# pitlover/Monocular-Depth-Estimation

Hardware: AMD Instinct MI355X
Metric: images/sec (train step) NYU 640x480 bs=8/GPU (higher is better)
Workload: dtype fp32; 1 GPU; NewCRFs Swin-L (large07) train step, NYU 480x640; model=NewCRFs-L07, global_batch=8, per_gpu_batch=8, num_accum=1, parallelism=dp1, reference_config=json/nyu/newcrfs/newcrfs_github_eval.json, matmul_precision=fp32, hipgraph=False

## Files before the change

### include/mdemi.h

```cpp
#ifndef MDEMI_H
#define MDEMI_H

#include <stddef.h>
#include <stdint.h>

#ifdef __cplusplus
extern "C" {
#endif

#define MDEMI_OK 0
#define MDEMI_EINVAL (-1)
#define MDEMI_ELAUNCH (-2)
#define MDEMI_EUNSUP (-3)
#define MDEMI_EWORKSPACE (-4)

const char* mdemi_last_error(void);
int mdemi_version(void);


#define MDEMI_L_KCONTIG 0
#define MDEMI_L_MNCONTIG 1
#define MDEMI_L_CONV 2
#define MDEMI_OP_NONE 0
#define MDEMI_OP_GELU 1
#define MDEMI_BIAS_NONE 0
#define MDEMI_BIAS_COL 1
#define MDEMI_BIAS_ROW 2
#define MDEMI_ACT_NONE 0
#define MDEMI_ACT_GELU 1
#define MDEMI_ACT_RELU 2
#define MDEMI_ACT_LEAKY 3
#define MDEMI_ACT_GELU_GRAD 4
#define MDEMI_ACT_SIGMOID 5
#define MDEMI_ACT_SILU 6
#define MDEMI_ACT_RELU_GRAD 7
#define MDEMI_ACT_SILU_GRAD 8
#define MDEMI_PAD_ZERO 0
#define MDEMI_PAD_REPLICATE 1

typedef struct mdemi_conv_geom {
  int32_t n, h, w, c;
  int32_t oh, ow;
  int32_t kh, kw, stride, pad;
  int32_t pad_mode;
  int32_t _reserved;
} mdemi_conv_geom;

typedef struct mdemi_gemm_desc {
  int32_t M, N, K, batch;
  const float* A; int64_t lda; int64_t a_bstride; int32_t a_layout; int32_t a_op;
  const float* B; int64_t ldb; int64_t b_bstride; int32_t b_layout; int32_t b_op;
  float* C; int64_t ldc; int64_t c_bstride;
  float alpha, beta;
  const float* bias; int32_t bias_mode; int32_t act;
  const float* aux; int64_t ldaux; int64_t aux_bstride;
  const float* residual; int64_t ldres; int64_t res_bstride;
  int32_t split_k; int32_t _pad0;
  void* workspace; int64_t workspace_bytes;
  mdemi_conv_geom conv;
  float* preact; int64_t ldpre; int64_t pre_bstride;
  float* rowsum_a;
  int32_t batch_inner; int32_t _pad1;
  int64_t a_bstride_inner, b_bstride_inner, c_bstride_inner;
  const float* row_scale; int64_t row_scale_group;
  const float* m_live; int64_t m_live_group;
  const float* k_live; int64_t k_live_group;
} mdemi_gemm_desc;

size_t mdemi_gemm_workspace_size(const mdemi_gemm_desc* d);
int mdemi_gemm_f32(const mdemi_gemm_desc* d, void* stream);
int mdemi_gemm_f32_pair(const mdemi_gemm_desc* d0, const mdemi_gemm_desc* d1, void* stream);
size_t mdemi_gemm_pair_workspace_size(const mdemi_gemm_desc* d0, const mdemi_gemm_desc* d1);
size_t mdemi_gemm_pair_workspace_offset(const mdemi_gemm_desc* d0);
int mdemi_gemm_pair_set_options(int32_t enabled, int32_t force_arm);
int mdemi_gemm_pair_enabled(void);
int mdemi_gemm_pair_last_arm(void);
int mdemi_gemm_bf16(const mdemi_gemm_desc* d, void* stream);
int mdemi_gemm_f32e(const mdemi_gemm_desc* d, void* stream);
int mdemi_gemm_bf16x(const mdemi_gemm_desc* d, const void* a16, const void* b16, void* c16, void* stream);
int mdemi_cast_bf16(const float* x, void* y, int64_t n, void* stream);
int mdemi_add16(const float* a, const float* b, float* y, void* y16, int64_t n, void* stream);
int mdemi_gemm_bf16x_supported(const mdemi_gemm_desc* d, const void* a16, const void* b16);
int mdemi_gemm_set_variant_b16(int32_t variant);
int mdemi_gemm_set_variant(int32_t variant, int32_t group_m);
int mdemi_gemm_set_variant_m16(int32_t variant);
int mdemi_gemm_set_options(int32_t tail_split, int32_t inline_reduce);

size_t mdemi_colsum_workspace_size(int64_t rows, int64_t cols);
int mdemi_colsum_f32(const float* x, int64_t rows, int64_t cols, int64_t ld,
                     float* out, int accumulate, void* workspace, void* stream);

int mdemi_headconv_fwd(const float* x, const float* w, const float* b, float* y, int32_t N,
                       int32_t H, int32_t W, int32_t C, int32_t K, int32_t pad, void* stream);
size_t mdemi_headconv_wgrad_workspace_size(int32_t N, int32_t H, int32_t W, int32_t C, int32_t K);
int mdemi_headconv_bwd(const float* dy, const float* x, const float* w, float* dx, float* dw,
                       float* db, int32_t N, int32_t H, int32_t W, int32_t C, int32_t K, int32_t pad,
                       void* workspace, void* stream);

int mdemi_binhead_fwd(const float* logits, const float* centers, float* pred,
                      float* stats, float* probs_out, int32_t B, int32_t K, int64_t HW,
                      int32_t do_softmax, void* stream);
size_t mdemi_binhead_bwd_workspace_size(int32_t B, int32_t K, int64_t HW);
int mdemi_binhead_bwd(const float* logits, const float* centers, const float* pred,
                      const float* stats, const float* dpred, float* dlogits,
                      float* dcenters, int32_t B, int32_t K, int64_t HW, int32_t do_softmax,
                      void* workspace, void* stream);

int mdemi_layernorm_fwd(const float* x, const float* gamma, const float* beta,
                        float* y, float* mean, float* rstd, int64_t rows, int32_t C,
                        float eps, void* stream);
int mdemi_layernorm_fwd16(const float* x, const float* gamma, const float* beta, float* y, void* y16,
                          float* mean, float* rstd, int64_t rows, int32_t C, float eps, void* stream);
size_t mdemi_layernorm_bwd_workspace_size(int64_t rows, int32_t C);
int mdemi_layernorm_bwd(const float* dy, const float* x, const float* mean,
                        const float* rstd, const float* gamma, float* dx,
                        float* dgamma, float* dbeta, int64_t rows, int32_t C,
                        int32_t accumulate_dx, void* workspace, void* stream);
int mdemi_layernorm_bwd_add(const float* dy, const float* x, const float* mean,
                            const float* rstd, const float* gamma, const float* dadd, float* dx,
                            float* dgamma, float* dbeta, int64_t rows, int32_t C,
                            void* workspace, void* stream);

typedef struct mdemi_winattn_desc {
  int32_t B, H, W, heads, head_dim, window, shift, _pad0;
  float scale;
  int32_t _pad1;
  const float* q; const float* k; int64_t qk_ld;
  const float* q_pad; const float* k_pad;
  const float* v; int64_t v_ld; const float* v_pad;
  const float* rpb_table;
  float* out; int64_t out_ld;
  float* lse;
  const float* dout;
  float* dq; float* dk; int64_t dqk_ld;
  float* dv; int64_t dv_ld;
  float* d_rpb_table;
  float* dq_pad; float* dk_pad; float* dv_pad;
  void* workspace; int64_t workspace_bytes;
  const float* sample_live;
} mdemi_winattn_desc;

size_t mdemi_winattn_fwd_workspace_size(const mdemi_winattn_desc* d);
int mdemi_winattn_fwd(const mdemi_winattn_desc* d, void* stream);
size_t mdemi_winattn_bwd_workspace_size(const mdemi_winattn_desc* d);
int mdemi_winattn_bwd(const mdemi_winattn_desc* d, void* stream);
int mdemi_winattn_bwd_bias(const mdemi_winattn_desc* d, const float* bias_expanded, void* stream);

size_t mdemi_silog_workspace_size(int32_t B, int64_t HW);
int mdemi_silog_fwd(const float* pred, const float* gt, float* loss, float* stats,
                    int32_t B, int64_t HW, float min_depth, float alpha, float beta,
                    int32_t per_image, int32_t unbiased, void* workspace, void* stream);
int mdemi_silog_bwd(const float* pred, const float* gt, const float* stats,
                    const float* dloss, float* dpred, int32_t B, int64_t HW,
                    float min_depth, float alpha, float beta, int32_t per_image,
                    int32_t unbiased, void* stream);

int mdemi_bilinear_fwd(const float* x, float* out, int32_t N, int32_t H, int32_t W,
                       int32_t C, int32_t OH, int32_t OW, int32_t align_corners,
                       float scale_h, float scale_w, int64_t in_cstride,
                       int64_t out_cstride, void* stream);
int mdemi_bilinear_bwd(const float* dout, float* dx, int32_t N, int32_t H, int32_t W,
                       int32_t C, int32_t OH, int32_t OW, int32_t align_corners,
                       float scale_h, float scale_w, int64_t dout_cstride,
                       int64_t dx_cstride, int32_t accumulate, void* stream);

int mdemi_nchw_to_nhwc(const float* x, float* y, int32_t N, int32_t C, int64_t HW, void* stream);
int mdemi_nhwc_to_nchw(const float* x, float* y, int32_t N, int32_t C, int64_t HW, void* stream);
int mdemi_pixel_shuffle_nhwc(const float* x, float* y, int32_t N, int32_t H, int32_t W,
                             int32_t C, int32_t r, int32_t inverse, void* stream);
int mdemi_patchify_nchw(const float* img, float* cols, int32_t N, int32_t C, int32_t H,
                        int32_t W, int32_t p, int32_t inverse, void* stream);

int mdemi_space_to_depth2(const float* x, float* y, int32_t N, int32_t H, int32_t W, int32_t C,
                          int32_t inverse, void* stream);
int mdemi_copy2d(const float* src, int64_t src_ld, float* dst, int64_t dst_ld, int64_t rows,
                 int64_t cols, int32_t accumulate, void* stream);

int mdemi_adaptive_avgpool_fwd(const float* x, float* y, int32_t N, int32_t H, int32_t W,
                               int32_t C, int32_t OH, int32_t OW, void* stream);
int mdemi_adaptive_avgpool_bwd(const float* dy, float* dx, int32_t N, int32_t H, int32_t W,
                               int32_t C, int32_t OH, int32_t OW, void* stream);

size_t mdemi_chnorm_workspace_size(int32_t N, int64_t HW, int32_t C, int32_t groups, int32_t is_bn);
int mdemi_chnorm_fwd(const float* x, const float* gamma, const float* beta, float* y,
                     float* mean, float* rstd, int32_t N, int64_t HW, int32_t C,
                     int32_t groups, int32_t is_bn, float eps, int32_t act,
                     void* workspace, void* stream);
int mdemi_chnorm_bwd(const float* dy, const float* x, const float* y, const float* mean,
                     const float* rstd, const float* gamma, const float* beta, float* dx,
                     float* dgamma, float* dbeta, int32_t N, int64_t HW, int32_t C,
                     int32_t groups, int32_t is_bn, int32_t act, void* workspace, void* stream);

int mdemi_chnorm_apply(const float* x, const float* gamma, const float* beta, const float* mean,
                       const float* rstd, float* y, int32_t N, int64_t HW, int32_t C, int32_t groups,
                       int32_t is_bn, int32_t act, void* stream);
int mdemi_bn_train_fwd(const float* x, const float* gamma, const float* beta, float* y, float* mean,
                       float* rstd, float* running_mean, float* running_var, int64_t* num_batches_tracked,
                       float momentum, int32_t N, int64_t HW, int32_t C, float eps, int32_t act,
                       void* workspace, void* stream);
int mdemi_bn_train_fwd16(const float* x, const float* gamma, const float* beta, float* y, void* y16,
                         float* mean, float* rstd, float* running_mean, float* running_var,
                         int64_t* num_batches_tracked, float momentum, int32_t N, int64_t HW, int32_t C,
                         float eps, int32_t act, void* workspace, void* stream);
size_t mdemi_bn_train_fwd_pooled_workspace_size(int32_t N, int64_t HW, int32_t C);
int mdemi_bn_train_fwd_pooled(const float* x, const float* gamma, const float* beta, float* y, void* y16,
                              float* pooled, float* mean, float* rstd, float* running_mean, float* running_var,
                              int64_t* num_batches_tracked, float momentum, int32_t N, int64_t HW, int32_t C,
                              float eps, int32_t act, void* workspace, void* stream);
int mdemi_chnorm_bwd16(const float* dy, const float* x, const float* y, const float* mean,
                       const float* rstd, const float* gamma, const float* beta, float* dx, void* dx16,
                       float* dgamma, float* dbeta, int32_t N, int64_t HW, int32_t C,
                       int32_t groups, int32_t is_bn, int32_t act, void* workspace, void* stream);
int mdemi_bn_frozen_bwd(const float* dy, const float* x, const float* mean, const float* rstd,
                        const float* gamma, const float* beta, float* dx, float* dgamma, float* dbeta,
                        int32_t N, int64_t HW, int32_t C, int32_t act, void* workspace, void* stream);
int mdemi_bn_running_update(const float* mean, const float* rstd, float* running_mean, float* running_var,
                            int64_t* num_batches_tracked, int32_t C, int64_t rows, float eps, float momentum,
                            void* stream);

#define MDEMI_EW_ADD 0
#define MDEMI_EW_SIGMOID_SCALE 1
#define MDEMI_EW_SIGMOID_SCALE_BWD 2
#define MDEMI_EW_AXPBY 3
#define MDEMI_EW_ACT_BWD 4
int mdemi_elementwise(int32_t op, const float* a, const float* b, float* y, int64_t n,
                      float s, float t, void* stream);
int mdemi_rowscale_add(const float* a, const float* b, const float* scale, float* y,
                       int64_t per_group, int64_t n, void* stream);

typedef struct mdemi_tensor_ref {
  float* param; float* grad; float* exp_avg; float* exp_avg_sq;
  int64_t numel; int32_t group;
  int32_t step_slot;
} mdemi_tensor_ref;

typedef struct mdemi_adamw_group {
  float lr, beta1, beta2, eps, weight_decay;
  int32_t _pad;
} mdemi_adamw_group;

int mdemi_multi_tensor_chunk(void);
size_t mdemi_grad_norm_workspace_size(int32_t nitems);
int mdemi_grad_sumsq(const mdemi_tensor_ref* tensors_dev, int32_t ntensors, int64_t nitems,
                     float grad_scale, float* sumsq, void* workspace, void* stream);
int mdemi_adamw_step(const mdemi_tensor_ref* tensors_dev, int32_t ntensors,
                     const mdemi_adamw_group* groups_host, int32_t ngroups,
                     const float* sumsq, float max_norm, float grad_scale, int32_t step,
                     int32_t* tensor_steps, int64_t nitems, void* workspace, void* stream);
int mdemi_adamw_step_dev(const mdemi_tensor_ref* tensors_dev, int32_t ntensors,
                         const mdemi_adamw_group* sched_dev, int32_t nsteps, int32_t ngroups,
                         int32_t* step_dev, int32_t* tensor_steps, const float* sumsq, float max_norm,
                         float grad_scale, int64_t nitems, void* workspace, void* stream);
int mdemi_adamw_step16(const mdemi_tensor_ref* tensors_dev, int32_t ntensors,
                       const mdemi_adamw_group* groups_host, int32_t ngroups,
                       const float* sumsq, float max_norm, float grad_scale, int32_t step,
                       int32_t* tensor_steps, int64_t nitems, void* const* param16_dev, void* workspace,
                       void* stream);
int mdemi_adamw_step_dev16(const mdemi_tensor_ref* tensors_dev, int32_t ntensors,
                           const mdemi_adamw_group* sched_dev, int32_t nsteps, int32_t ngroups,
                           int32_t* step_dev, int32_t* tensor_steps, const float* sumsq, float max_norm,
                           float grad_scale, int64_t nitems, void* const* param16_dev, void* workspace,
                           void* stream);

#ifdef __cplusplus
}
#endif
#endif
```

### monocular-depth-estimation_amd/csrc/winattn.hip

```cpp
#include "common.h"

namespace mdemi {

struct WinGeom {
  int B, H, W, Hp, Wp, nWh, nWw, shift, heads;
};

template <int WS>
struct Win {
  int b, wy, wx;
  __device__ Win(const WinGeom& g, int win) {
    wx = win % g.nWw;
    const int t = win / g.nWw;
    wy = t % g.nWh;
    b = t / g.nWh;
  }
  __device__ int row(const WinGeom& g, int t) const {
    const int py = wy * WS + t / WS, px = wx * WS + t % WS;
    int oy = py + g.shift, ox = px + g.shift;
    if (oy >= g.Hp) oy -= g.Hp;
    if (ox >= g.Wp) ox -= g.Wp;
    if (oy >= g.H || ox >= g.W) return -1;
    return (b * g.H + oy) * g.W + ox;
  }
  __device__ int region(const WinGeom& g, int t) const {
    const int py = wy * WS + t / WS, px = wx * WS + t % WS;
    const int rh = py < g.Hp - WS ? 0 : (py < g.Hp - g.shift ? 1 : 2);
    const int rw = px < g.Wp - WS ? 0 : (px < g.Wp - g.shift ? 1 : 2);
    return rh * 3 + rw;
  }
};

template <int WS>
__device__ __forceinline__ int rpb_index(int i, int j) {
  return (i / WS - j / WS + WS - 1) * (2 * WS - 1) + (i % WS - j % WS + WS - 1);
}

template <int HD>
__device__ __forceinline__ void load_row(float4 (&dst)[HD / 4], const float* src) {
#pragma unroll
  for (int q = 0; q < HD / 4; ++q) dst[q] = reinterpret_cast<const float4*>(src)[q];
}

__device__ __forceinline__ float4 ld_tok4(const float* base, int64_t ld, int row, const float* pad, int off) {
  if (row >= 0) return *reinterpret_cast<const float4*>(base + (int64_t)row * ld + off);
  if (pad) return *reinterpret_cast<const float4*>(pad + off);
  return make_float4(0.f, 0.f, 0.f, 0.f);
}

__device__ float g_wa_zero[128];

__device__ __forceinline__ const float* tok_src(const float* base, int64_t ld, int row, const float* pad, bool real) {
  const float* padsrc = pad ? pad : g_wa_zero;
  return !real ? g_wa_zero : (row >= 0 ? base + (int64_t)row * ld : padsrc);
}

__device__ __forceinline__ float dot4(const float4& a, const float4& b) {
  return fmaf(a.x, b.x, fmaf(a.y, b.y, fmaf(a.z, b.z, a.w * b.w)));
}

struct WinParams {
  WinGeom g;
  float scale;
  const float* q; const float* k; int64_t qk_ld;
  const float* q_pad; const float* k_pad;
  const float* v; int64_t v_ld; const float* v_pad;
  const float* rpb;
  float* out; int64_t out_ld;
  float* lse;
  const float* dout;
  float* dq; float* dk; int64_t dqk_ld;
  float* dv; int64_t dv_ld;
  float* partial;
  int off32;
  const float* live;
};

constexpr int WA_WAVES = 4, WA_NP = 64, WA_HD = 32, WA_N = 49, WA_T = 169;
typedef float wa_f16x __attribute__((ext_vector_type(16)));

__device__ __forceinline__ float f4c(const float4& v, int c) {
  return c == 0 ? v.x : (c == 1 ? v.y : (c == 2 ? v.z : v.w));
}
__device__ __forceinline__ wa_f16x mfma32(float a, float b, wa_f16x c) {
  return __builtin_amdgcn_mfma_f32_32x32x2f32(a, b, c, 0, 0, 0);
}
__device__ __forceinline__ int acc_row(int r, int h) { return (r & 3) + 8 * (r >> 2) + 4 * h; }

__device__ __forceinline__ void load_frag(float4 (&f)[4], const float* base, int64_t ld, int row, const float* pad,
                                          bool real, int col0, int h, float scale) {
  const float* src = tok_src(base, ld, row, pad, real);
  src = src == g_wa_zero ? src : src + col0;
#pragma unroll
  for (int g4 = 0; g4 < 4; ++g4) {
    float4 v = *reinterpret_cast<const float4*>(src + 8 * g4 + 4 * h);
    v.x *= scale; v.y *= scale; v.z *= scale; v.w *= scale;
    f[g4] = v;
  }
}

__device__ __forceinline__ void load_bias(wa_f16x (&acc)[2][2], const float* img, int lane) {
#pragma unroll
  for (int a = 0; a < 2; ++a)
#pragma unroll
    for (int b = 0; b < 2; ++b) {
      const float4* src = reinterpret_cast<const float4*>(img + ((a * 2 + b) * 64 + lane) * 16);
#pragma unroll
      for (int q4 = 0; q4 < 4; ++q4) {
        const float4 v = src[q4];
        acc[a][b][4 * q4 + 0] = v.x; acc[a][b][4 * q4 + 1] = v.y;
        acc[a][b][4 * q4 + 2] = v.z; acc[a][b][4 * q4 + 3] = v.w;
      }
    }
}

__device__ __forceinline__ void mma_hd(wa_f16x (&acc)[2][2], const float4 (&fa)[2][4], const float4 (&fb)[2][4]) {
#pragma unroll
  for (int g4 = 0; g4 < 4; ++g4)
#pragma unroll
    for (int c = 0; c < 4; ++c)
#pragma unroll
      for (int a = 0; a < 2; ++a)
#pragma unroll
        for (int b = 0; b < 2; ++b) acc[a][b] = mfma32(f4c(fa[a][g4], c), f4c(fb[b][g4], c), acc[a][b]);
}

__device__ __forceinline__ void mma_tok(wa_f16x (&out)[2], const float (*rows)[WA_HD], const wa_f16x (&acc)[2][2],
                                        int l31, int h) {
#pragma unroll
  for (int t = 0; t < 2; ++t)
#pragma unroll
    for (int s = 0; s < (t == 0 ? 16 : 12); ++s) {
      const float a = rows[t * 32 + acc_row(s, h)][l31];
#pragma unroll
      for (int n = 0; n < 2; ++n) out[n] = mfma32(a, acc[t][n][s], out[n]);
    }
}

__device__ __forceinline__ void wave_lds_sync() {
  __builtin_amdgcn_fence(__ATOMIC_RELEASE, "wavefront");
  __builtin_amdgcn_wave_barrier();
  __builtin_amdgcn_fence(__ATOMIC_ACQUIRE, "wavefront");
}

struct WaItem {
  int item, win, hh;
};
__device__ __forceinline__ WaItem wa_item(const WinParams& p) {
  WaItem it;
  it.item = blockIdx.x * WA_WAVES + (threadIdx.x >> 6);
  it.win = it.item / p.g.heads;
  it.hh = it.item % p.g.heads;
  return it;
}

__device__ __forceinline__ bool wa_dead(const WinParams& p, int b) { return p.live && p.live[b] == 0.f; }
__device__ __forceinline__ void wa_zero_rows(const WinGeom& g, const Win<7>& w, float* base, int64_t ld, int col0,
                                             int lane) {
  for (int e = lane; e < WA_N * (WA_HD / 4); e += 64) {
    const int row = w.row(g, e >> 3);
    if (row >= 0)
      *reinterpret_cast<float4*>(base + (int64_t)row * ld + col0 + 4 * (e & 7)) = make_float4(0.f, 0.f, 0.f, 0.f);
  }
}

__device__ __forceinline__ bool wa_regions(const WinParams& p, const Win<7>& w, int8_t* reg, int lane) {
  const bool border = p.g.shift > 0 && (w.wy == p.g.nWh - 1 || w.wx == p.g.nWw - 1);
  if (border) reg[lane] = lane < WA_N ? (int8_t)w.region(p.g, lane) : (int8_t)0;
  return border;
}

template <int WS, int HD>
__global__ __launch_bounds__(256) void winattn_fwd_kernel(WinParams p, const float* __restrict__ biasT, int nitems) {
  static_assert(WS == 7 && HD == WA_HD, "MFMA window attention is built for 7x7 windows, head_dim 32");
  __shared__ float Vs[WA_WAVES][WA_NP][WA_HD];
  __shared__ int8_t regs[WA_WAVES][WA_NP];
  const WinGeom& g = p.g;
  const int lane = threadIdx.x & 63, wv = threadIdx.x >> 6, l31 = lane & 31, h = lane >> 5;
  const WaItem it = wa_item(p);
  if (it.item >= nitems) return;
  const Win<WS> w(g, it.win);
  const int col0 = it.hh * HD;
  if (wa_dead(p, w.b)) {
    wa_zero_rows(g, w, p.out, p.out_ld, col0, lane);
    if (p.lse && lane < WA_N) p.lse[(int64_t)it.item * WA_N + lane] = 0.f;
    return;
  }
  for (int e = lane; e < WA_NP * HD / 4; e += 64) {
    const int tok = e >> 3, c4 = e & 7;
    const float4 v = tok < WA_N ? ld_tok4(p.v, p.v_ld, w.row(g, tok), p.v_pad, col0 + 4 * c4)
                                : make_float4(0.f, 0.f, 0.f, 0.f);
    *reinterpret_cast<float4*>(&Vs[wv][tok][4 * c4]) = v;
  }
  const bool border = wa_regions(p, w, regs[wv], lane);
  wa_f16x s[2][2];
  load_bias(s, biasT + (size_t)it.hh * 4096, lane);
  {
    float4 kf[2][4], qf[2][4];
#pragma unroll
    for (int t = 0; t < 2; ++t) {
      const int tok = t * 32 + l31;
      const bool real = tok < WA_N;
      const int row = real ? w.row(g, tok) : -1;
      load_frag(kf[t], p.k, p.qk_ld, row, p.k_pad, real, col0, h, 1.f);
      load_frag(qf[t], p.q, p.qk_ld, row, p.q_pad, real, col0, h, p.scale);
    }
    mma_hd(s, kf, qf);
  }
  wave_lds_sync();
  if (border) {
#pragma unroll
    for (int n = 0; n < 2; ++n) {
      const int rq = regs[wv][n * 32 + l31];
#pragma unroll
      for (int t = 0; t < 2; ++t)
#pragma unroll
        for (int r = 0; r < 16; ++r)
          if (regs[wv][t * 32 + acc_row(r, h)] != rq) s[t][n][r] -= 100.f;
    }
  }
  float lse[2];
#pragma unroll
  for (int n = 0; n < 2; ++n) {
    float m = -INFINITY;
#pragma unroll
    for (int t = 0; t < 2; ++t)
#pragma unroll
      for (int r = 0; r < 16; ++r) m = fmaxf(m, s[t][n][r]);
    m = fmaxf(m, __shfl_xor(m, 32, 64));
    float l = 0.f;
#pragma unroll
    for (int t = 0; t < 2; ++t)
#pragma unroll
      for (int r = 0; r < 16; ++r) {
        const float e = __expf(s[t][n][r] - m);
        s[t][n][r] = e;
        l += e;
      }
    l += __shfl_xor(l, 32, 64);
    const float inv = 1.f / l;
#pragma unroll
    for (int t = 0; t < 2; ++t)
#pragma unroll
      for (int r = 0; r < 16; ++r) s[t][n][r] *= inv;
    lse[n] = m + __logf(l);
  }
  wa_f16x o[2];
#pragma unroll
  for (int n = 0; n < 2; ++n)
#pragma unroll
    for (int r = 0; r < 16; ++r) o[n][r] = 0.f;
  mma_tok(o, Vs[wv], s, l31, h);
#pragma unroll
  for (int n = 0; n < 2; ++n) {
    const int q = n * 32 + l31;
    if (q >= WA_N) continue;
    const int row = w.row(g, q);
    if (p.lse && h == 0) p.lse[(int64_t)it.item * WA_N + q] = row >= 0 ? lse[n] : INFINITY;
    if (row < 0) continue;
    float* dst = p.out + (int64_t)row * p.out_ld + col0;
#pragma unroll
    for (int a = 0; a < 4; ++a)
      *reinterpret_cast<float4*>(dst + 8 * a + 4 * h) =
          make_float4(o[n][4 * a], o[n][4 * a + 1], o[n][4 * a + 2], o[n][4 * a + 3]);
  }
}

#ifdef WA_OCC3
constexpr int WA_TR = 56, WA_TP = 57;
#else
constexpr int WA_TR = WA_NP, WA_TP = WA_NP + 1;
#endif

__device__ __forceinline__ float col_val(const float* base, int64_t ld, const float* pad, int row, int col) {
  const float* src = row >= 0 ? base + (int64_t)row * ld + col : ((row == -1 && pad) ? pad + col : g_wa_zero + (col & 31));
  return *src;
}

__host__ __device__ constexpr int key_tab(int key) { return (key / 7) * 13 + key % 7; }

__host__ __device__ constexpr int acc_tok_kind(int ti, int r) {
  return (ti * 32 + (r & 3) + 8 * (r >> 2) + 4 >= WA_N) ? ((ti * 32 + (r & 3) + 8 * (r >> 2) >= WA_N) ? 2 : 1) : 0;
}
__host__ __device__ constexpr int pair_tok_kind(int j) { return 2 * j + 1 >= WA_N ? (2 * j >= WA_N ? 2 : 1) : 0; }

template <bool FAST>
__device__ __forceinline__ void fetch_pairs(float (&c)[25], const float* base, int64_t ld, const float* pad,
                                            const int* rt, int col0, int l31, int h, float scale) {
  if (FAST) {
    const float* cb = base + col0 + l31;
#pragma unroll
    for (int j = 0; j < 25; ++j) {
      const int kind = pair_tok_kind(j);
      const float v = cb[__umul24((unsigned)rt[kind ? 2 * j : 2 * j + h], (unsigned)ld)];
      c[j] = (kind && h) ? 0.f : scale * v;
    }
  } else {
#pragma unroll
    for (int j = 0; j < 25; ++j) c[j] = scale * col_val(base, ld, pad, rt[2 * j + h], col0 + l31);
  }
}

template <bool FAST>
__device__ __forceinline__ void fetch_keys(float (&c)[2][16], const float* base, int64_t ld, const float* pad,
                                           const int* rt, int col0, int l31, int h) {
  if (FAST) {
    const float* cb = base + col0 + l31;
#pragma unroll
    for (int t = 0; t < 2; ++t)
#pragma unroll
      for (int r = 0; r < 16; ++r) {
        const int kind = acc_tok_kind(t, r);
        if (kind == 2) {
          c[t][r] = 0.f;
          continue;
        }
        const float v = cb[__umul24((unsigned)rt[kind ? t * 32 + acc_row(r, 0) : t * 32 + acc_row(r, h)], (unsigned)ld)];
        c[t][r] = (kind && h) ? 0.f : v;
      }
  } else {
#pragma unroll
    for (int t = 0; t < 2; ++t)
#pragma unroll
      for (int r = 0; r < 16; ++r) c[t][r] = col_val(base, ld, pad, rt[t * 32 + acc_row(r, h)], col0 + l31);
  }
}

template <int WS, int HD>
#ifdef WA_OCC3
#define WA_BWD_OCC 3
#else
#define WA_BWD_OCC 2
#endif
__global__ __launch_bounds__(256) __attribute__((amdgpu_waves_per_eu(WA_BWD_OCC, WA_BWD_OCC))) void winattn_bwd_kernel(
    WinParams p, const float* __restrict__ biasT, int nitems) {
  __shared__ float tbuf[WA_WAVES][WA_TR][WA_TP];
  __shared__ float padk[WA_WAVES][WA_HD], padv[WA_WAVES][WA_HD];
  __shared__ int8_t regs[WA_WAVES][WA_NP];
  __shared__ int rowtab[WA_WAVES][WA_NP];
  const WinGeom& g = p.g;
  const int lane = threadIdx.x & 63, wv = threadIdx.x >> 6, l31 = lane & 31, h = lane >> 5;
  const WaItem it = wa_item(p);
  if (it.item >= nitems) return;
  const Win<WS> w(g, it.win);
  const int col0 = it.hh * HD;
  if (wa_dead(p, w.b)) {
    wa_zero_rows(g, w, p.dq, p.dqk_ld, col0, lane);
    wa_zero_rows(g, w, p.dk, p.dqk_ld, col0, lane);
    wa_zero_rows(g, w, p.dv, p.dv_ld, col0, lane);
    float* P = p.partial + (int64_t)it.item * (WA_T + 2 * HD);
    for (int e = lane; e < WA_T + 2 * HD; e += 64) P[e] = 0.f;
    return;
  }
  float lse[2];
#pragma unroll
  for (int n = 0; n < 2; ++n) {
    const int q = n * 32 + l31;
    lse[n] = (q < WA_N) ? p.lse[(int64_t)it.item * WA_N + q] : INFINITY;
  }
  const int myrow = lane < WA_N ? w.row(g, lane) : -2;
  rowtab[wv][lane] = myrow;
  if (lane < HD) { padk[wv][lane] = 0.f; padv[wv][lane] = 0.f; }
  const bool border = wa_regions(p, w, regs[wv], lane);
  const bool fast = p.off32 && __ballot(myrow == -1) == 0;

  wa_f16x s[2][2], dp[2][2];
  load_bias(s, biasT + (size_t)it.hh * 4096, lane);
  int trow[2];
  bool treal[2];
  {
    float4 kf[2][4], qf[2][4];
#pragma unroll
    for (int t = 0; t < 2; ++t) {
      const int tok = t * 32 + l31;
      treal[t] = tok < WA_N;
      trow[t] = treal[t] ? w.row(g, tok) : -1;
      load_frag(kf[t], p.k, p.qk_ld, trow[t], p.k_pad, treal[t], col0, h, 1.f);
      load_frag(qf[t], p.q, p.qk_ld, trow[t], p.q_pad, treal[t], col0, h, p.scale);
    }
    mma_hd(s, kf, qf);
  }
  wave_lds_sync();
  if (border) {
#pragma unroll
    for (int n = 0; n < 2; ++n) {
      const int rq = regs[wv][n * 32 + l31];
#pragma unroll
      for (int t = 0; t < 2; ++t)
#pragma unroll
        for (int r = 0; r < 16; ++r)
          if (regs[wv][t * 32 + acc_row(r, h)] != rq) s[t][n][r] -= 100.f;
    }
  }
#pragma unroll
  for (int n = 0; n < 2; ++n)
#pragma unroll
    for (int t = 0; t < 2; ++t)
#pragma unroll
      for (int r = 0; r < 16; ++r) s[t][n][r] = __expf(s[t][n][r] - lse[n]);
  auto to_lds = [&](const wa_f16x (&x)[2][2]) {
#pragma unroll
    for (int t = 0; t < 2; ++t)
#pragma unroll
      for (int n = 0; n < 2; ++n)
#pragma unroll
        for (int r = 0; r < 16; ++r) {
#ifdef WA_OCC3
          if (t * 32 + acc_row(r, 0) >= WA_TR || (n == 1 && l31 >= WA_TP - 32)) continue;
#endif
          tbuf[wv][t * 32 + acc_row(r, h)][n * 32 + l31] = x[t][n][r];
        }
  };
  auto key_side = [&](const float (&colv)[25], float* gbase, int64_t gld, float* padacc) {
    wa_f16x acc[2];
#pragma unroll
    for (int ti = 0; ti < 2; ++ti)
#pragma unroll
      for (int r = 0; r < 16; ++r) acc[ti][r] = 0.f;
#pragma unroll
    for (int j = 0; j < 25; ++j)
#pragma unroll
      for (int ti = 0; ti < 2; ++ti) acc[ti] = mfma32(tbuf[wv][ti * 32 + l31][2 * j + h], colv[j], acc[ti]);
    if (fast) {
      float* gb = gbase + col0 + l31;
      const int* rt = rowtab[wv];
#pragma unroll
      for (int ti = 0; ti < 2; ++ti)
#pragma unroll
        for (int r = 0; r < 16; ++r) {
          const int kind = acc_tok_kind(ti, r);
          if (kind == 2 || (kind == 1 && h)) continue;
          gb[__umul24((unsigned)rt[ti * 32 + acc_row(r, h)], (unsigned)gld)] = acc[ti][r];
        }
      return;
    }
#pragma unroll
    for (int ti = 0; ti < 2; ++ti)
#pragma unroll
      for (int r = 0; r < 16; ++r) {
        const int row = rowtab[wv][ti * 32 + acc_row(r, h)];
        if (row >= 0) gbase[(int64_t)row * gld + col0 + l31] = acc[ti][r];
        else if (row == -1) atomicAdd(&padacc[l31], acc[ti][r]);
      }
  };
  {
    to_lds(s);
    wave_lds_sync();
    float dc[25];
    if (fast) fetch_pairs<true>(dc, p.dout, p.out_ld, nullptr, rowtab[wv], col0, l31, h, 1.f);
    else fetch_pairs<false>(dc, p.dout, p.out_ld, nullptr, rowtab[wv], col0, l31, h, 1.f);
    key_side(dc, p.dv, p.dv_ld, padv[wv]);
  }
  float D[2];
  {
    float4 vf[2][4], df[2][4];
#pragma unroll
    for (int t = 0; t < 2; ++t) {
      const bool qo = treal[t] && trow[t] >= 0;
      load_frag(vf[t], p.v, p.v_ld, trow[t], p.v_pad, treal[t], col0, h, 1.f);
      load_frag(df[t], p.dout, p.out_ld, trow[t], nullptr, qo, col0, h, 1.f);
      float4 of[4];
      load_frag(of, p.out, p.out_ld, trow[t], nullptr, qo, col0, h, 1.f);
      float part = 0.f;
#pragma unroll
      for (int g4 = 0; g4 < 4; ++g4) part += dot4(df[t][g4], of[g4]);
      D[t] = part + __shfl_xor(part, 32, 64);
    }
#pragma unroll
    for (int a = 0; a < 2; ++a)
#pragma unroll
      for (int b = 0; b < 2; ++b)
#pragma unroll
        for (int r = 0; r < 16; ++r) dp[a][b][r] = 0.f;
    mma_hd(dp, vf, df);
  }
#pragma unroll
  for (int n = 0; n < 2; ++n)
#pragma unroll
    for (int t = 0; t < 2; ++t)
#pragma unroll
      for (int r = 0; r < 16; ++r) {
        float pr;
#ifdef WA_OCC3
        if (t * 32 + acc_row(r, 0) >= WA_TR) pr = 0.f;
        else if (n == 1) pr = l31 < WA_TP - 32 ? tbuf[wv][t * 32 + acc_row(r, h)][32 + min(l31, WA_TP - 33)] : 0.f;
        else
#endif
        pr = tbuf[wv][t * 32 + acc_row(r, h)][n * 32 + l31];
        dp[t][n][r] = pr * (dp[t][n][r] - D[n]);
      }
  float kc[2][16];
  if (fast) fetch_keys<true>(kc, p.k, p.qk_ld, p.k_pad, rowtab[wv], col0, l31, h);
  else fetch_keys<false>(kc, p.k, p.qk_ld, p.k_pad, rowtab[wv], col0, l31, h);
  wave_lds_sync();
  to_lds(dp);
  wave_lds_sync();
  float qc[25];
  if (fast) fetch_pairs<true>(qc, p.q, p.qk_ld, p.q_pad, rowtab[wv], col0, l31, h, p.scale);
  else fetch_pairs<false>(qc, p.q, p.qk_ld, p.q_pad, rowtab[wv], col0, l31, h, p.scale);
  {
    wa_f16x dq[2];
#pragma unroll
    for (int n = 0; n < 2; ++n)
#pragma unroll
      for (int r = 0; r < 16; ++r) dq[n][r] = 0.f;
#pragma unroll
    for (int t = 0; t < 2; ++t)
#pragma unroll
      for (int r = 0; r < (t == 0 ? 16 : 12); ++r)
#pragma unroll
        for (int n = 0; n < 2; ++n)
          dq[n] = mfma32(kc[t][r], tbuf[wv][t * 32 + acc_row(r, h)][n * 32 + l31], dq[n]);
#pragma unroll
    for (int n = 0; n < 2; ++n) {
      if (!treal[n] || trow[n] < 0) continue;
      float* dst = p.dq + (int64_t)trow[n] * p.dqk_ld + col0;
#pragma unroll
      for (int a = 0; a < 4; ++a)
        *reinterpret_cast<float4*>(dst + 8 * a + 4 * h) =
            make_float4(dq[n][4 * a] * p.scale, dq[n][4 * a + 1] * p.scale, dq[n][4 * a + 2] * p.scale,
                        dq[n][4 * a + 3] * p.scale);
    }
  }
  key_side(qc, p.dk, p.dqk_ld, padk[wv]);
  float E[13];
#pragma unroll
  for (int e = 0; e < 13; ++e) E[e] = 0.f;
  const int sky = lane / WS, sqy = lane - sky * WS;
  if (lane < WA_N) {
    const float* blk = &tbuf[wv][sky * WS][sqy * WS];
#pragma unroll
    for (int kx = 0; kx < WS; ++kx)
#pragma unroll
      for (int qx = 0; qx < WS; ++qx) E[qx - kx + WS - 1] += blk[kx * WA_TP + qx];
  }
  wave_lds_sync();
  constexpr int ND = 2 * WS - 1;
  float* Eb = &tbuf[wv][0][0];
  if (lane < WA_N) {
#pragma unroll
    for (int e = 0; e < ND; ++e) Eb[lane * ND + e] = E[e];
  }
  wave_lds_sync();
  float* P = p.partial + (int64_t)it.item * (WA_T + 2 * HD);
  for (int e = lane; e < WA_T; e += 64) {
    const int dy = e / ND - (WS - 1), dxi = e % ND;
    const int ky0 = max(0, -dy), ky1 = min(WS - 1, WS - 1 - dy);
    float acc = 0.f;
    for (int ky = ky0; ky <= ky1; ++ky) acc += Eb[(ky * WS + ky + dy) * ND + dxi];
    P[e] = acc;
  }
  if (lane < HD) {
    P[WA_T + lane] = padk[wv][lane];
    P[WA_T + HD + lane] = padv[wv][lane];
  }
}

__global__ __launch_bounds__(256) void wa_bias_kernel(const float* __restrict__ rpb, int heads, float* biasT,
                                                      float* biasN) {
  const int e = blockIdx.x * 256 + threadIdx.x;
  if (e >= heads * 4096) return;
  const int hh = e >> 12, rem = e & 4095;
  const int tile = rem >> 10, lane = (rem >> 4) & 63, r = rem & 15;
  const int row = (tile >> 1) * 32 + acc_row(r, lane >> 5), col = (tile & 1) * 32 + (lane & 31);
  auto val = [&](int q, int key) {
    if (key >= WA_N) return -INFINITY;
    if (q >= WA_N) return 0.f;
    return rpb[rpb_index<7>(q, key) * heads + hh];
  };
  if (biasT) biasT[e] = val(col, row);
  if (biasN) biasN[e] = val(row, col);
}

template <int WS, int HD>
__global__ void winattn_bwd_scatter(const float* __restrict__ sums, int heads, float* d_rpb, float* dk_pad,
                                    float* dv_pad, float* dq_pad) {
  constexpr int T = (2 * WS - 1) * (2 * WS - 1), R = T + 2 * HD;
  const int e = blockIdx.x * blockDim.x + threadIdx.x;
  if (e >= heads * R) return;
  const int h = e / R, t = e % R;
  const float s = sums[e];
  if (t < T) d_rpb[t * heads + h] = s;
  else if (t < T + HD) { if (dk_pad) dk_pad[h * HD + t - T] = s; }
  else if (dv_pad) dv_pad[h * HD + t - T - HD] = s;
  if (dq_pad && t < HD) dq_pad[h * HD + t] = 0.f;
}

static int make_params(const mdemi_winattn_desc* d, WinParams& p, int& nwin) {
  MDEMI_REQUIRE(d, "winattn: null descriptor");
  MDEMI_REQUIRE(d->B > 0 && d->H > 0 && d->W > 0 && d->heads > 0, "winattn: bad sizes");
  MDEMI_REQUIRE(d->window == 7 && d->head_dim == 32, "winattn: only window 7 / head_dim 32 are built (got %d/%d)",
                d->window, d->head_dim);
  MDEMI_REQUIRE(d->shift >= 0 && d->shift < d->window, "winattn: bad shift %d", d->shift);
  MDEMI_REQUIRE(d->q && d->k && d->v && d->rpb_table, "winattn: null input");
  MDEMI_REQUIRE(d->qk_ld % 4 == 0 && d->v_ld % 4 == 0 && d->out_ld % 4 == 0, "winattn: row strides must be %% 4");
  const int ws = d->window;
  p.g.B = d->B; p.g.H = d->H; p.g.W = d->W;
  p.g.Hp = (d->H + ws - 1) / ws * ws; p.g.Wp = (d->W + ws - 1) / ws * ws;
  p.g.nWh = p.g.Hp / ws; p.g.nWw = p.g.Wp / ws;
  p.g.shift = d->shift; p.g.heads = d->heads;
  p.scale = d->scale;
  p.q = d->q; p.k = d->k; p.qk_ld = d->qk_ld; p.q_pad = d->q_pad; p.k_pad = d->k_pad;
  p.v = d->v; p.v_ld = d->v_ld; p.v_pad = d->v_pad;
  p.rpb = d->rpb_table;
  p.out = d->out; p.out_ld = d->out_ld;
  p.lse = d->lse;
  p.dout = d->dout; p.dq = d->dq; p.dk = d->dk; p.dqk_ld = d->dqk_ld; p.dv = d->dv; p.dv_ld = d->dv_ld;
  p.partial = (float*)d->workspace;
  p.live = d->sample_live;
  {
    const int64_t rows = (int64_t)d->B * d->H * d->W;
    const int64_t lds[4] = {d->qk_ld, d->out_ld, d->dqk_ld, d->dv_ld};
    bool ok = rows < (1 << 24);
    for (int64_t ld : lds) ok = ok && ld >= 0 && ld < (1 << 24) && rows * ld < (int64_t(1) << 32);
    p.off32 = ok;
  }
  nwin = d->B * p.g.nWh * p.g.nWw;
  return MDEMI_OK;
}

}

using namespace mdemi;

static int wa_items(const mdemi_winattn_desc* d, int nwin) { return nwin * d->heads; }
static size_t wa_bias_bytes(const mdemi_winattn_desc* d) { return (size_t)d->heads * 4096 * sizeof(float); }

extern "C" size_t mdemi_winattn_fwd_workspace_size(const mdemi_winattn_desc* d) {
  WinParams p;
  int nwin;
  if (make_params(d, p, nwin)) return 0;
  return wa_bias_bytes(d);
}

extern "C" int mdemi_winattn_fwd(const mdemi_winattn_desc* d, void* stream) {
  WinParams p;
  int nwin;
  int rc = make_params(d, p, nwin);
  if (rc) return rc;
  MDEMI_REQUIRE(d->out, "winattn_fwd: null out");
  if (!d->workspace || (size_t)d->workspace_bytes < wa_bias_bytes(d)) {
    set_error("winattn_fwd: needs %zu workspace bytes", wa_bias_bytes(d));
    return MDEMI_EWORKSPACE;
  }
  hipStream_t st = (hipStream_t)stream;
  float* biasT = (float*)d->workspace;
  hipLaunchKernelGGL(wa_bias_kernel, dim3(d->heads * 16), dim3(256), 0, st, d->rpb_table, d->heads, biasT,
                     (float*)nullptr);
  const int nitems = wa_items(d, nwin);
  hipLaunchKernelGGL((winattn_fwd_kernel<7, 32>), dim3(cdiv(nitems, WA_WAVES)), dim3(64 * WA_WAVES), 0, st, p,
                     (const float*)biasT, nitems);
  return check_launch("winattn_fwd");
}

static size_t wa_part_bytes(int items, int R) { return align_up((size_t)items * R * 4, 256); }
extern "C" size_t mdemi_winattn_bwd_workspace_size(const mdemi_winattn_desc* d) {
  WinParams p;
  int nwin;
  if (make_params(d, p, nwin)) return 0;
  const int R = WA_T + 2 * WA_HD;
  const int items = wa_items(d, nwin);
  return wa_part_bytes(items, R) + wa_bias_bytes(d) + align_up((size_t)d->heads * R * 4, 256) +
         colsum_ws_bytes(nwin, (int64_t)d->heads * R);
}

extern "C" int mdemi_winattn_bwd(const mdemi_winattn_desc* d, void* stream) {
  return mdemi_winattn_bwd_bias(d, nullptr, stream);
}

extern "C" int mdemi_winattn_bwd_bias(const mdemi_winattn_desc* d, const float* bias_expanded, void* stream) {
  WinParams p;
  int nwin;
  int rc = make_params(d, p, nwin);
  if (rc) return rc;
  MDEMI_REQUIRE(d->dout && d->dq && d->dk && d->dv && d->d_rpb_table, "winattn_bwd: null gradient buffer");
  MDEMI_REQUIRE(d->out && d->lse, "winattn_bwd: needs the forward output and its saved lse");
  MDEMI_REQUIRE(d->dqk_ld % 4 == 0 && d->dv_ld % 4 == 0, "winattn_bwd: gradient strides must be %% 4");
  const size_t need = mdemi_winattn_bwd_workspace_size(d);
  if (!d->workspace || (size_t)d->workspace_bytes < need) {
    set_error("winattn_bwd: needs %zu workspace bytes", need);
    return MDEMI_EWORKSPACE;
  }
  hipStream_t st = (hipStream_t)stream;
  const int R = WA_T + 2 * WA_HD;
  const int items = wa_items(d, nwin);
  char* ws = (char*)d->workspace;
  p.partial = (float*)ws;
  float* biasT = (float*)(ws + wa_part_bytes(items, R));
  float* sums = (float*)((char*)biasT + wa_bias_bytes(d));
  void* cws = (char*)sums + align_up((size_t)d->heads * R * 4, 256);
  if (bias_expanded)
    biasT = const_cast<float*>(bias_expanded);
  else
    hipLaunchKernelGGL(wa_bias_kernel, dim3(d->heads * 16), dim3(256), 0, st, d->rpb_table, d->heads, biasT,
                       (float*)nullptr);
  hipLaunchKernelGGL((winattn_bwd_kernel<7, 32>), dim3((unsigned)cdiv(items, WA_WAVES)), dim3(64 * WA_WAVES), 0, st,
                     p, (const float*)biasT, items);
  int rc2 = colsum_launch(p.partial, nwin, (int64_t)d->heads * R, (int64_t)d->heads * R, sums, 0, cws, st);
  if (rc2) return rc2;
  hipLaunchKernelGGL((winattn_bwd_scatter<7, 32>), dim3((d->heads * R + 255) / 256), dim3(256), 0, st, sums, d->heads,
                     d->d_rpb_table, d->dk_pad, d->dv_pad, d->dq_pad);
  return check_launch("winattn_bwd");
}
```

### monocular-depth-estimation_amd/mdemi/_lib.py

```python
from __future__ import annotations

import ctypes
import os
import threading

import torch

_HERE = os.path.dirname(os.path.abspath(__file__))
LIB_PATH = os.environ.get("MDEMI_LIB") or os.path.join(_HERE, "libmdemi.so")
HEADER_PATH = os.path.abspath(os.path.join(_HERE, "..", "..", "include", "mdemi.h"))
HEADER_PATHS = [HEADER_PATH, os.path.abspath(os.path.join(_HERE, "..", "..", "include", "mdemi_ext.h"))]

c_float_p = ctypes.POINTER(ctypes.c_float)
vp = ctypes.c_void_p
i32 = ctypes.c_int32
i64 = ctypes.c_int64
f32 = ctypes.c_float
sz = ctypes.c_size_t

L_KCONTIG, L_MNCONTIG, L_CONV = 0, 1, 2
OP_NONE, OP_GELU = 0, 1
BIAS_NONE, BIAS_COL, BIAS_ROW = 0, 1, 2
ACT_NONE, ACT_GELU, ACT_RELU, ACT_LEAKY, ACT_GELU_GRAD, ACT_SIGMOID = 0, 1, 2, 3, 4, 5
ACT_SILU, ACT_RELU_GRAD, ACT_SILU_GRAD = 6, 7, 8
ACT_GRAD_OF = {ACT_GELU: ACT_GELU_GRAD, ACT_RELU: ACT_RELU_GRAD, ACT_SILU: ACT_SILU_GRAD}
BINS_RELU, BINS_ELU = 0, 1
WL_OHWI, WL_OIHW, WL_DGRAD = 0, 1, 2
ALIGN_MEDIAN, ALIGN_LSTSQ, ALIGN_LSTSQ_DISP = 1, 2, 3
PAD_ZERO, PAD_REPLICATE = 0, 1
EW_ADD, EW_SIGMOID_SCALE, EW_SIGMOID_SCALE_BWD, EW_AXPBY, EW_ACT_BWD = 0, 1, 2, 3, 4


class ConvGeom(ctypes.Structure):
    _fields_ = [(n, i32) for n in ("n", "h", "w", "c", "oh", "ow", "kh", "kw", "stride", "pad",
                                   "pad_mode", "_reserved")]


class GemmDesc(ctypes.Structure):
    _fields_ = [
        ("M", i32), ("N", i32), ("K", i32), ("batch", i32),
        ("A", vp), ("lda", i64), ("a_bstride", i64), ("a_layout", i32), ("a_op", i32),
        ("B", vp), ("ldb", i64), ("b_bstride", i64), ("b_layout", i32), ("b_op", i32),
        ("C", vp), ("ldc", i64), ("c_bstride", i64),
        ("alpha", f32), ("beta", f32),
        ("bias", vp), ("bias_mode", i32), ("act", i32),
        ("aux", vp), ("ldaux", i64), ("aux_bstride", i64),
        ("residual", vp), ("ldres", i64), ("res_bstride", i64),
        ("split_k", i32), ("_pad0", i32),
        ("workspace", vp), ("workspace_bytes", i64),
        ("conv", ConvGeom),
        ("preact", vp), ("ldpre", i64), ("pre_bstride", i64),
        ("rowsum_a", vp),
        ("batch_inner", i32), ("_pad1", i32),
        ("a_bstride_inner", i64), ("b_bstride_inner", i64), ("c_bstride_inner", i64),
        ("row_scale", vp), ("row_scale_group", i64),
        ("m_live", vp), ("m_live_group", i64),
        ("k_live", vp), ("k_live_group", i64),
    ]


class WinAttnDesc(ctypes.Structure):
    _fields_ = [
        ("B", i32), ("H", i32), ("W", i32), ("heads", i32), ("head_dim", i32), ("window", i32),
        ("shift", i32), ("_pad0", i32),
        ("scale", f32), ("_pad1", i32),
        ("q", vp), ("k", vp), ("qk_ld", i64),
        ("q_pad", vp), ("k_pad", vp),
        ("v", vp), ("v_ld", i64), ("v_pad", vp),
        ("rpb_table", vp),
        ("out", vp), ("out_ld", i64),
        ("lse", vp),
        ("dout", vp),
        ("dq", vp), ("dk", vp), ("dqk_ld", i64),
        ("dv", vp), ("dv_ld", i64),
        ("d_rpb_table", vp),
        ("dq_pad", vp), ("dk_pad", vp), ("dv_pad", vp),
        ("workspace", vp), ("workspace_bytes", i64),
        ("sample_live", vp),
    ]


class TensorRef(ctypes.Structure):
    _fields_ = [("param", vp), ("grad", vp), ("exp_avg", vp), ("exp_avg_sq", vp),
                ("numel", i64), ("group", i32), ("step_slot", i32)]


class AdamWGroup(ctypes.Structure):
    _fields_ = [("lr", f32), ("beta1", f32), ("beta2", f32), ("eps", f32), ("weight_decay", f32),
                ("_pad", i32)]


STEP_LOSS_NONFINITE, STEP_GRAD_NONFINITE = 1, 2


class StepRecord(ctypes.Structure):
    _fields_ = [("loss", f32), ("grad_sumsq", f32), ("index", i32), ("flags", ctypes.c_uint32)]


class TelemetryState(ctypes.Structure):
    _fields_ = [("pushed", i32), ("nonfinite_steps", i32), ("first_nonfinite", i32), ("_pad", i32)]


class GuardState(ctypes.Structure):
    _fields_ = [("skipped", i32), ("consecutive", i32), ("last_skipped", i32), ("calls", i32)]


class EmaState(ctypes.Structure):
    _fields_ = [("updates", i32)]


AUG_MAX_SPANS = 8


class AugSample(ctypes.Structure):
    _fields_ = [("affine", ctypes.c_double * 6), ("fixed", i32 * 6), ("rotate", i32), ("crop_x", i32),
                ("crop_y", i32), ("flip", i32), ("gamma", f32), ("brightness", f32), ("color", f32 * 3),
                ("n_rows", i32), ("n_cols", i32), ("mask_keep", i32), ("rows", (i32 * 2) * AUG_MAX_SPANS),
                ("cols", (i32 * 2) * AUG_MAX_SPANS)]


_SIGS = {
    "mdemi_last_error": (ctypes.c_char_p, []),
    "mdemi_version": (ctypes.c_int, []),
    "mdemi_gemm_workspace_size": (sz, [ctypes.POINTER(GemmDesc)]),
    "mdemi_gemm_f32": (ctypes.c_int, [ctypes.POINTER(GemmDesc), vp]),
    "mdemi_gemm_bf16": (ctypes.c_int, [ctypes.POINTER(GemmDesc), vp]),
    "mdemi_gemm_f32e": (ctypes.c_int, [ctypes.POINTER(GemmDesc), vp]),
    "mdemi_gemm_set_variant": (ctypes.c_int, [i32, i32]),
    "mdemi_gemm_set_variant_m16": (ctypes.c_int, [i32]),
    "mdemi_gemm_bf16x": (ctypes.c_int, [ctypes.POINTER(GemmDesc), vp, vp, vp, vp]),
    "mdemi_gemm_bf16x_supported": (ctypes.c_int, [ctypes.POINTER(GemmDesc), vp, vp]),
    "mdemi_gemm_set_variant_b16": (ctypes.c_int, [i32]),
    "mdemi_cast_bf16": (ctypes.c_int, [vp, vp, i64, vp]),
    "mdemi_add16": (ctypes.c_int, [vp, vp, vp, vp, i64, vp]),
    "mdemi_bn_train_fwd16": (ctypes.c_int, [vp, vp, vp, vp, vp, vp, vp, vp, vp, vp, f32, i32, i64, i32, f32, i32, vp,
                                            vp]),
    "mdemi_bn_train_fwd_pooled_workspace_size": (sz, [i32, i64, i32]),
    "mdemi_bn_train_fwd_pooled": (ctypes.c_int, [vp, vp, vp, vp, vp, vp, vp, vp, vp, vp, vp, f32, i32, i64, i32, f32, i32,
                                                 vp, vp]),
    "mdemi_chnorm_bwd16": (ctypes.c_int, [vp, vp, vp, vp, vp, vp, vp, vp, vp, vp, vp, i32, i64, i32, i32, i32, i32,
                                          vp, vp]),
    "mdemi_chan_scale16": (ctypes.c_int, [vp, vp, vp, vp, vp, i32, i64, i32, vp]),
    "mdemi_gemm_set_options": (ctypes.c_int, [i32, i32]),
    "mdemi_gemm_f32_pair": (ctypes.c_int, [ctypes.POINTER(GemmDesc), ctypes.POINTER(GemmDesc), vp]),
    "mdemi_gemm_pair_workspace_size": (sz, [ctypes.POINTER(GemmDesc), ctypes.POINTER(GemmDesc)]),
    "mdemi_gemm_pair_workspace_offset": (sz, [ctypes.POINTER(GemmDesc)]),
    "mdemi_gemm_pair_set_options": (ctypes.c_int, [i32, i32]),
    "mdemi_gemm_pair_enabled": (ctypes.c_int, []),
    "mdemi_gemm_pair_last_arm": (ctypes.c_int, []),
    "mdemi_colsum_workspace_size": (sz, [i64, i64]),
    "mdemi_colsum_f32": (ctypes.c_int, [vp, i64, i64, i64, vp, ctypes.c_int, vp, vp]),
    "mdemi_headconv_fwd": (ctypes.c_int, [vp, vp, vp, vp, i32, i32, i32, i32, i32, i32, vp]),
    "mdemi_headconv_wgrad_workspace_size": (sz, [i32, i32, i32, i32, i32]),
    "mdemi_headconv_bwd": (ctypes.c_int, [vp, vp, vp, vp, vp, vp, i32, i32, i32, i32, i32, i32, vp, vp]),
    "mdemi_binhead_fwd": (ctypes.c_int, [vp, vp, vp, vp, vp, i32, i32, i64, i32, vp]),
    "mdemi_binhead_bwd_workspace_size": (sz, [i32, i32, i64]),
    "mdemi_binhead_bwd": (ctypes.c_int, [vp, vp, vp, vp, vp, vp, vp, i32, i32, i64, i32, vp, vp]),
    "mdemi_layernorm_fwd": (ctypes.c_int, [vp, vp, vp, vp, vp, vp, i64, i32, f32, vp]),
    "mdemi_layernorm_fwd16": (ctypes.c_int, [vp, vp, vp, vp, vp, vp, vp, i64, i32, f32, vp]),
    "mdemi_layernorm_bwd_workspace_size": (sz, [i64, i32]),
    "mdemi_layernorm_bwd": (ctypes.c_int, [vp, vp, vp, vp, vp, vp, vp, vp, i64, i32, i32, vp, vp]),
    "mdemi_layernorm_bwd_add": (ctypes.c_int, [vp, vp, vp, vp, vp, vp, vp, vp, vp, i64, i32, vp, vp]),
    "mdemi_winattn_fwd_workspace_size": (sz, [ctypes.POINTER(WinAttnDesc)]),
    "mdemi_winattn_fwd": (ctypes.c_int, [ctypes.POINTER(WinAttnDesc), vp]),
    "mdemi_winattn_bwd_workspace_size": (sz, [ctypes.POINTER(WinAttnDesc)]),
    "mdemi_winattn_bwd": (ctypes.c_int, [ctypes.POINTER(WinAttnDesc), vp]),
    "mdemi_winattn_bwd_bias": (ctypes.c_int, [ctypes.POINTER(WinAttnDesc), vp, vp]),
    "mdemi_silog_workspace_size": (sz, [i32, i64]),
    "mdemi_silog_fwd": (ctypes.c_int, [vp, vp, vp, vp, i32, i64, f32, f32, f32, i32, i32, vp, vp]),
    "mdemi_silog_bwd": (ctypes.c_int, [vp, vp, vp, vp, vp, i32, i64, f32, f32, f32, i32, i32, vp]),
    "mdemi_bilinear_fwd": (ctypes.c_int, [vp, vp, i32, i32, i32, i32, i32, i32, i32, f32, f32, i64, i64, vp]),
    "mdemi_bilinear_bwd": (ctypes.c_int, [vp, vp, i32, i32, i32, i32, i32, i32, i32, f32, f32, i64, i64, i32, vp]),
    "mdemi_nchw_to_nhwc": (ctypes.c_int, [vp, vp, i32, i32, i64, vp]),
    "mdemi_nhwc_to_nchw": (ctypes.c_int, [vp, vp, i32, i32, i64, vp]),
    "mdemi_pixel_shuffle_nhwc": (ctypes.c_int, [vp, vp, i32, i32, i32, i32, i32, i32, vp]),
    "mdemi_patchify_nchw": (ctypes.c_int, [vp, vp, i32, i32, i32, i32, i32, i32, vp]),
    "mdemi_adaptive_avgpool_fwd": (ctypes.c_int, [vp, vp, i32, i32, i32, i32, i32, i32, vp]),
    "mdemi_adaptive_avgpool_bwd": (ctypes.c_int, [vp, vp, i32, i32, i32, i32, i32, i32, vp]),
    "mdemi_chnorm_workspace_size": (sz, [i32, i64, i32, i32, i32]),
    "mdemi_chnorm_fwd": (ctypes.c_int, [vp, vp, vp, vp, vp, vp, i32, i64, i32, i32, i32, f32, i32, vp, vp]),
    "mdemi_chnorm_bwd": (ctypes.c_int, [vp, vp, vp, vp, vp, vp, vp, vp, vp, vp, i32, i64, i32, i32, i32, i32,
                                        vp, vp]),
    "mdemi_elementwise": (ctypes.c_int, [i32, vp, vp, vp, i64, f32, f32, vp]),
    "mdemi_rowscale_add": (ctypes.c_int, [vp, vp, vp, vp, i64, i64, vp]),
    "mdemi_space_to_depth2": (ctypes.c_int, [vp, vp, i32, i32, i32, i32, i32, vp]),
    "mdemi_copy2d": (ctypes.c_int, [vp, i64, vp, i64, i64, i64, i32, vp]),
    "mdemi_chnorm_apply": (ctypes.c_int, [vp, vp, vp, vp, vp, vp, i32, i64, i32, i32, i32, i32, vp]),
    "mdemi_bn_frozen_bwd": (ctypes.c_int, [vp, vp, vp, vp, vp, vp, vp, vp, vp, i32, i64, i32, i32, vp, vp]),
    "mdemi_bn_train_fwd": (ctypes.c_int, [vp, vp, vp, vp, vp, vp, vp, vp, vp, f32, i32, i64, i32, f32, i32, vp, vp]),
    "mdemi_bn_running_update": (ctypes.c_int, [vp, vp, vp, vp, vp, i32, i64, f32, f32, vp]),
    "mdemi_multi_tensor_chunk": (ctypes.c_int, []),
    "mdemi_grad_norm_workspace_size": (sz, [i32]),
    "mdemi_grad_sumsq": (ctypes.c_int, [vp, i32, i64, f32, vp, vp, vp]),
    "mdemi_adamw_step": (ctypes.c_int, [vp, i32, ctypes.POINTER(AdamWGroup), i32, vp, f32, f32, i32, vp, i64, vp, vp]),
    "mdemi_adamw_step_dev": (ctypes.c_int, [vp, i32, vp, i32, i32, vp, vp, vp, f32, f32, i64, vp, vp]),
    "mdemi_adamw_step16": (ctypes.c_int, [vp, i32, ctypes.POINTER(AdamWGroup), i32, vp, f32, f32, i32, vp, i64, vp, vp,
                                          vp]),
    "mdemi_adamw_step_dev16": (ctypes.c_int, [vp, i32, vp, i32, i32, vp, vp, vp, f32, f32, i64, vp, vp, vp]),
    "mdemi_dwconv_fwd": (ctypes.c_int, [vp, vp, vp, i32, i32, i32, i32, i32, i32, i32, i32, i32, i32, vp]),
    "mdemi_dwconv_bwd_workspace_size": (sz, [i32, i32, i32, i32, i32]),
    "mdemi_dwconv_bwd": (ctypes.c_int, [vp, vp, vp, vp, vp, i32, i32, i32, i32, i32, i32, i32, i32, i32, i32, vp,
                                        vp]),
    "mdemi_spatial_reduce_workspace_size": (sz, [i32, i64, i32]),
    "mdemi_spatial_reduce": (ctypes.c_int, [vp, vp, vp, i32, i64, i32, f32, vp, vp]),
    "mdemi_chan_scale": (ctypes.c_int, [vp, vp, vp, vp, i32, i64, i32, vp]),
    "mdemi_se_gate_fwd": (ctypes.c_int, [vp, vp, vp, vp, vp, vp, vp, i32, i32, i32, vp]),
    "mdemi_se_gate_bwd_workspace_size": (sz, [i32, i32, i32]),
    "mdemi_se_gate_bwd": (ctypes.c_int, [vp, vp, vp, vp, vp, vp, vp, vp, vp, vp, vp, i32, i32, i32, f32, vp, vp]),
    "mdemi_softmax_fwd": (ctypes.c_int, [vp, vp, i64, i32, f32, vp]),
    "mdemi_softmax_bwd": (ctypes.c_int, [vp, vp, vp, i64, i32, f32, i32, vp]),
    "mdemi_softmax_fwd16": (ctypes.c_int, [vp, vp, vp, i64, i32, f32, vp]),
    "mdemi_softmax_bwd16": (ctypes.c_int, [vp, vp, vp, vp, i64, i32, f32, i32, vp]),
    "mdemi_act_fwd": (ctypes.c_int, [vp, vp, i64, i32, vp]),
    "mdemi_dropout": (ctypes.c_int, [vp, vp, i64, f32, ctypes.c_uint64, ctypes.c_uint64, vp]),
    "mdemi_dropout_dev": (ctypes.c_int, [vp, vp, i64, f32, vp, ctypes.c_uint64, ctypes.c_uint64, vp]),
    "mdemi_dropout_dev16": (ctypes.c_int, [vp, vp, vp, i64, f32, vp, ctypes.c_uint64, ctypes.c_uint64, vp]),
    "mdemi_softmax_fwd_drop16": (ctypes.c_int, [vp, vp, vp, i64, i32, f32, f32, vp, ctypes.c_uint64, ctypes.c_uint64,
                                                vp]),
    "mdemi_binhead_nhwc_fwd": (ctypes.c_int, [vp, vp, vp, vp, i32, i64, i32, vp]),
    "mdemi_binhead_nhwc_bwd_workspace_size": (sz, [i32, i64, i32]),
    "mdemi_binhead_nhwc_bwd": (ctypes.c_int, [vp, vp, vp, vp, vp, vp, vp, i32, i64, i32, vp, vp]),
    "mdemi_bins_fwd": (ctypes.c_int, [vp, vp, vp, vp, i32, i32, i32, f32, f32, vp]),
    "mdemi_bins_bwd": (ctypes.c_int, [vp, vp, vp, vp, vp, i32, i32, i32, f32, f32, vp]),
    "mdemi_nchw_to_nhwc_pad": (ctypes.c_int, [vp, vp, i32, i32, i64, i32, vp]),
    "mdemi_unpatchify_nhwc": (ctypes.c_int, [vp, vp, i32, i32, i32, i32, i32, i32, i32, vp]),
    "mdemi_pad_fold_replicate": (ctypes.c_int, [vp, vp, i32, i32, i32, i32, i32, vp]),
    "mdemi_depth_metrics_workspace_size": (sz, [i32, i32, i32]),
    "mdemi_depth_metrics": (ctypes.c_int, [vp, vp, i32, i32, i32, i32, i32, i32, i32, f32, f32, i32, vp, vp, vp]),
    "mdemi_depth_align_workspace_size": (sz, [i32, i32, i32, i32]),
    "mdemi_depth_align": (ctypes.c_int, [vp, vp, i32, i32, i32, i32, i32, i32, i32, f32, f32, i32, vp, vp, vp]),
    "mdemi_depth_metrics_aligned": (ctypes.c_int, [vp, vp, i32, i32, i32, i32, i32, i32, i32, f32, f32, i32, i32, vp,
                                                   vp, vp, vp, vp]),
    "mdemi_flip_w": (ctypes.c_int, [vp, vp, i64, i32, vp]),
    "mdemi_flip_avg_w": (ctypes.c_int, [vp, vp, vp, i64, i32, vp]),
    "mdemi_depth_export": (ctypes.c_int, [vp, i32, i32, i32, i32, i32, f32, f32, vp, f32, vp, vp, vp, vp]),
    "mdemi_bins_chamfer_workspace_size": (sz, [i32, i32, i64]),
    "mdemi_bins_chamfer_fwd": (ctypes.c_int, [vp, vp, i32, i32, i32, i64, f32, vp, vp, vp, vp]),
    "mdemi_bins_chamfer_bwd": (ctypes.c_int, [vp, vp, vp, i32, i32, i32, vp]),
    "mdemi_conv_weight_layout": (ctypes.c_int, [vp, vp, i32, i32, i32, i32, i32, vp]),
    "mdemi_conv_weight_layout16": (ctypes.c_int, [vp, vp, vp, i32, i32, i32, i32, i32, vp]),
    "mdemi_augment": (ctypes.c_int, [vp, vp, i32, i32, i32, i32, i32, i32, i32, i32, i32, vp, i32, i32, i32,
                                     f32, f32, vp, vp, vp]),
    "mdemi_window_shuffle": (ctypes.c_int, [vp, vp, vp, i32, i32, i32, i32, i32, i32, i32, vp]),
    "mdemi_window_shuffle_i32": (ctypes.c_int, [vp, vp, i32, i32, i32, i32, i32, vp]),
    "mdemi_ordered_softmax_fwd": (ctypes.c_int, [vp, vp, vp, vp, i32, i32, i32, i32, f32, vp]),
    "mdemi_ordered_softmax_bwd_workspace_size": (sz, [i32, i32, i32]),
    "mdemi_ordered_softmax_bwd": (ctypes.c_int, [vp, vp, vp, vp, vp, i32, i32, i32, i32, f32, vp, vp]),
    "mdemi_glu_fwd": (ctypes.c_int, [vp, vp, i64, i32, vp]),
    "mdemi_glu_bwd": (ctypes.c_int, [vp, vp, vp, i64, i32, vp]),
    "mdemi_pad_replicate": (ctypes.c_int, [vp, vp, i32, i32, i32, i32, i32, i32, i32, i32, i32, vp]),
    "mdemi_param_sumsq": (ctypes.c_int, [vp, i32, i64, vp, vp, vp]),
    "mdemi_telemetry_push": (ctypes.c_int, [vp, i32, vp, vp, vp, vp]),
    "mdemi_adamw_step_guarded16": (ctypes.c_int, [vp, i32, ctypes.POINTER(AdamWGroup), i32, vp, f32, f32, vp, i64, vp,
                                                  vp, vp, vp]),
    "mdemi_adamw_step_dev_guarded16": (ctypes.c_int, [vp, i32, vp, i32, i32, vp, vp, vp, f32, f32, i64, vp, vp, vp,
                                                      vp]),
    "mdemi_adamw_step_ema16": (ctypes.c_int, [vp, i32, ctypes.POINTER(AdamWGroup), i32, vp, f32, f32, i32, vp, i64, vp,
                                              vp, f32, i32, vp, vp, vp, vp]),
    "mdemi_adamw_step_dev_ema16": (ctypes.c_int, [vp, i32, vp, i32, i32, vp, vp, vp, f32, f32, i64, vp, vp, f32, i32,
                                                  vp, vp, vp, vp]),
    "mdemi_gradmatch_workspace_size": (sz, [i32, i32, i32]),
    "mdemi_gradmatch_fwd": (ctypes.c_int, [vp, vp, vp, vp, i32, i32, i32, f32, i32, i32, vp, vp]),
    "mdemi_gradmatch_bwd": (ctypes.c_int, [vp, vp, vp, vp, vp, i32, i32, i32, f32, i32, vp]),
}

_lib = None
_lock = threading.Lock()


class MdemiLibraryError(RuntimeError):
    pass


def load():
    global _lib
    if _lib is not None:
        return _lib
    with _lock:
        if _lib is not None:
            return _lib
        if not os.path.exists(LIB_PATH):
            raise MdemiLibraryError(
                f"libmdemi.so not found at {LIB_PATH}; build it with "
                "`make -C monocular-depth-estimation_amd/csrc` (or __graft_entry__.build())")
        lib = ctypes.CDLL(LIB_PATH)
        for name, (res, args) in _SIGS.items():
            fn = getattr(lib, name, None)
            if fn is None:
                if os.environ.get("MDEMI_LIB"):
                    continue
                raise MdemiLibraryError(f"{LIB_PATH} does not export {name}")
            fn.restype = res
            fn.argtypes = args
        _lib = lib
    return _lib


def exported_symbols():
    return list(_SIGS.keys())


def check(rc: int, what: str) -> None:
    if rc != 0:
        msg = load().mdemi_last_error().decode(errors="replace")
        raise RuntimeError(f"mdemi {what} failed (rc={rc}): {msg}")


def call(name: str, *args):
    rc = getattr(load(), name)(*args)
    check(rc, name)


def ptr(t) -> int | None:
    if t is None:
        return None
    return t.data_ptr()


def stream() -> int:
    return torch.cuda.current_stream().cuda_stream


_ws: dict = {}
_ws_retired: list = []
_graph_captured = False


def note_graph_capture() -> None:
    global _graph_captured
    _graph_captured = True


def workspace(nbytes: int, device=None, slot: int = 0) -> torch.Tensor:
    if device is None:
        device = torch.device("cuda", torch.cuda.current_device())
    key = (device.index if device.index is not None else torch.cuda.current_device(), slot)
    buf = _ws.get(key)
    nbytes = max(int(nbytes), 256)
    capturing = torch.cuda.is_current_stream_capturing()
    if capturing:
        note_graph_capture()
    if buf is None or buf.numel() < nbytes:
        if capturing:
            raise RuntimeError(f"mdemi: workspace slot {slot} must grow to {nbytes} bytes during hipGraph capture; "
                               "run the captured step eagerly first (warm-up) so every workspace is sized")
        if buf is not None:
            if _graph_captured:
                _ws_retired.append(buf)
            else:
                torch.cuda.synchronize(device)
        buf = torch.empty(int(nbytes * 1.25) + 4096, dtype=torch.uint8, device=device)
        _ws[key] = buf
    return buf
```

Measured before the change: 63.10 images/sec.

## Make window-attention kernels persistent per head with LDS-staged bias

Window attention forward and backward now launch a grid sized to CU count times a target occupancy, one workgroup per (slot, head), instead of one workgroup per four (window, head) items. Each workgroup stages its head's relative-position bias into LDS once, then loops over windows, so every window reads the bias from LDS rather than global memory. The forward kernel gets a waves-per-EU attribute, and the backward kernel now always uses the trimmed 56-row transpose buffer that was previously behind an optional build flag. The trade-off is more LDS per workgroup, a fixed occupancy target, and possible tail imbalance when the window count does not divide evenly across slots.

```diff
diff --git a/include/mdemi.h b/include/mdemi.h
--- a/include/mdemi.h
+++ b/include/mdemi.h
@@ -145,6 +145,7 @@
 size_t mdemi_winattn_bwd_workspace_size(const mdemi_winattn_desc* d);
 int mdemi_winattn_bwd(const mdemi_winattn_desc* d, void* stream);
 int mdemi_winattn_bwd_bias(const mdemi_winattn_desc* d, const float* bias_expanded, void* stream);
+void mdemi_winattn_set_max_workgroups(int n);
 
 size_t mdemi_silog_workspace_size(int32_t B, int64_t HW);
 int mdemi_silog_fwd(const float* pred, const float* gt, float* loss, float* stats,
diff --git a/monocular-depth-estimation_amd/csrc/wa_plan.h b/monocular-depth-estimation_amd/csrc/wa_plan.h
--- /dev/null
+++ b/monocular-depth-estimation_amd/csrc/wa_plan.h
@@ -0,0 +1,40 @@
+#pragma once
+
+#ifdef __HIPCC__
+#define MDEMI_WA_HD __host__ __device__ __forceinline__
+#else
+#define MDEMI_WA_HD inline
+#endif
+
+namespace mdemi {
+
+constexpr int WA_WAVES = 4;
+constexpr int WA_FWD_WG_PER_CU = 3, WA_BWD_WG_PER_CU = 2;
+
+struct WaPlan {
+  int nwin, heads;
+  int slots;
+  int grid;
+};
+
+inline WaPlan wa_plan(int nwin, int heads, int max_wg) {
+  WaPlan pl;
+  pl.nwin = nwin;
+  pl.heads = heads;
+  const int need = (nwin + WA_WAVES - 1) / WA_WAVES;
+  int slots = max_wg / heads;
+  if (slots < 1) slots = 1;
+  pl.slots = slots < need ? slots : need;
+  pl.grid = pl.slots * heads;
+  return pl;
+}
+
+inline int wa_default_max_wg(int cus, int wg_per_cu, int forced) { return forced > 0 ? forced : cus * wg_per_cu; }
+
+MDEMI_WA_HD int wa_head(int wg, int heads) { return wg % heads; }
+MDEMI_WA_HD int wa_slot(int wg, int heads) { return wg / heads; }
+MDEMI_WA_HD int wa_first_win(int slot, int wave) { return slot * WA_WAVES + wave; }
+MDEMI_WA_HD int wa_win_stride(int slots) { return slots * WA_WAVES; }
+MDEMI_WA_HD int wa_item_index(int win, int heads, int head) { return win * heads + head; }
+
+}
diff --git a/monocular-depth-estimation_amd/csrc/winattn.hip b/monocular-depth-estimation_amd/csrc/winattn.hip
--- a/monocular-depth-estimation_amd/csrc/winattn.hip
+++ b/monocular-depth-estimation_amd/csrc/winattn.hip
@@ -1,4 +1,5 @@
 #include "common.h"
+#include "wa_plan.h"
 
 namespace mdemi {
 
@@ -76,7 +77,7 @@
   const float* live;
 };
 
-constexpr int WA_WAVES = 4, WA_NP = 64, WA_HD = 32, WA_N = 49, WA_T = 169;
+constexpr int WA_NP = 64, WA_HD = 32, WA_N = 49, WA_T = 169;
 typedef float wa_f16x __attribute__((ext_vector_type(16)));
 
 __device__ __forceinline__ float f4c(const float4& v, int c) {
@@ -99,15 +100,22 @@
   }
 }
 
-__device__ __forceinline__ void load_bias(wa_f16x (&acc)[2][2], const float* img, int lane) {
+constexpr int WA_BIAS_F4 = 4 * 64 * 4;
+__device__ __forceinline__ void stage_bias(float (*img_lds)[64][4], const float* img) {
+  for (int e = threadIdx.x; e < WA_BIAS_F4; e += 64 * WA_WAVES) {
+    const int ab = e >> 8, ln = (e >> 2) & 63, q4 = e & 3;
+    *reinterpret_cast<float4*>(img_lds[ab * 4 + q4][ln]) = reinterpret_cast<const float4*>(img)[e];
+  }
+}
+
+__device__ __forceinline__ void load_bias(wa_f16x (&acc)[2][2], const float (*img_lds)[64][4], int lane) {
 #pragma unroll
   for (int a = 0; a < 2; ++a)
 #pragma unroll
     for (int b = 0; b < 2; ++b) {
-      const float4* src = reinterpret_cast<const float4*>(img + ((a * 2 + b) * 64 + lane) * 16);
 #pragma unroll
       for (int q4 = 0; q4 < 4; ++q4) {
-        const float4 v = src[q4];
+        const float4 v = *reinterpret_cast<const float4*>(img_lds[(a * 2 + b) * 4 + q4][lane]);
         acc[a][b][4 * q4 + 0] = v.x; acc[a][b][4 * q4 + 1] = v.y;
         acc[a][b][4 * q4 + 2] = v.z; acc[a][b][4 * q4 + 3] = v.w;
       }
@@ -141,17 +149,6 @@
   __builtin_amdgcn_fence(__ATOMIC_RELEASE, "wavefront");
   __builtin_amdgcn_wave_barrier();
   __builtin_amdgcn_fence(__ATOMIC_ACQUIRE, "wavefront");
-}
-
-struct WaItem {
-  int item, win, hh;
-};
-__device__ __forceinline__ WaItem wa_item(const WinParams& p) {
-  WaItem it;
-  it.item = blockIdx.x * WA_WAVES + (threadIdx.x >> 6);
-  it.win = it.item / p.g.heads;
-  it.hh = it.item % p.g.heads;
-  return it;
 }
 
 __device__ __forceinline__ bool wa_dead(const WinParams& p, int b) { return p.live && p.live[b] == 0.f; }
@@ -171,109 +168,114 @@
 }
 
 template <int WS, int HD>
-__global__ __launch_bounds__(256) void winattn_fwd_kernel(WinParams p, const float* __restrict__ biasT, int nitems) {
+__global__ __launch_bounds__(256) __attribute__((amdgpu_waves_per_eu(WA_FWD_WG_PER_CU, WA_FWD_WG_PER_CU))) void
+winattn_fwd_kernel(WinParams p, const float* __restrict__ biasT, int nwin, int slots) {
   static_assert(WS == 7 && HD == WA_HD, "MFMA window attention is built for 7x7 windows, head_dim 32");
   __shared__ float Vs[WA_WAVES][WA_NP][WA_HD];
+  __shared__ float Bs[16][64][4];
   __shared__ int8_t regs[WA_WAVES][WA_NP];
   const WinGeom& g = p.g;
   const int lane = threadIdx.x & 63, wv = threadIdx.x >> 6, l31 = lane & 31, h = lane >> 5;
-  const WaItem it = wa_item(p);
-  if (it.item >= nitems) return;
-  const Win<WS> w(g, it.win);
-  const int col0 = it.hh * HD;
-  if (wa_dead(p, w.b)) {
-    wa_zero_rows(g, w, p.out, p.out_ld, col0, lane);
-    if (p.lse && lane < WA_N) p.lse[(int64_t)it.item * WA_N + lane] = 0.f;
-    return;
-  }
-  for (int e = lane; e < WA_NP * HD / 4; e += 64) {
-    const int tok = e >> 3, c4 = e & 7;
-    const float4 v = tok < WA_N ? ld_tok4(p.v, p.v_ld, w.row(g, tok), p.v_pad, col0 + 4 * c4)
-                                : make_float4(0.f, 0.f, 0.f, 0.f);
-    *reinterpret_cast<float4*>(&Vs[wv][tok][4 * c4]) = v;
-  }
-  const bool border = wa_regions(p, w, regs[wv], lane);
-  wa_f16x s[2][2];
-  load_bias(s, biasT + (size_t)it.hh * 4096, lane);
-  {
-    float4 kf[2][4], qf[2][4];
-#pragma unroll
-    for (int t = 0; t < 2; ++t) {
-      const int tok = t * 32 + l31;
-      const bool real = tok < WA_N;
-      const int row = real ? w.row(g, tok) : -1;
-      load_frag(kf[t], p.k, p.qk_ld, row, p.k_pad, real, col0, h, 1.f);
-      load_frag(qf[t], p.q, p.qk_ld, row, p.q_pad, real, col0, h, p.scale);
-    }
-    mma_hd(s, kf, qf);
-  }
-  wave_lds_sync();
-  if (border) {
+  const int hh = wa_head(blockIdx.x, g.heads), slot = wa_slot(blockIdx.x, g.heads);
+  const int col0 = hh * HD;
+  stage_bias(Bs, biasT + (size_t)hh * 4096);
+  __syncthreads();
+  for (int win = wa_first_win(slot, wv); win < nwin; win += wa_win_stride(slots)) {
+    const int item = wa_item_index(win, g.heads, hh);
+    const Win<WS> w(g, win);
+    if (wa_dead(p, w.b)) {
+      wa_zero_rows(g, w, p.out, p.out_ld, col0, lane);
+      if (p.lse && lane < WA_N) p.lse[(int64_t)item * WA_N + lane] = 0.f;
+      continue;
+    }
+    wave_lds_sync();
+    for (int e = lane; e < WA_NP * HD / 4; e += 64) {
+      const int tok = e >> 3, c4 = e & 7;
+      const float4 v = tok < WA_N ? ld_tok4(p.v, p.v_ld, w.row(g, tok), p.v_pad, col0 + 4 * c4)
+                                  : make_float4(0.f, 0.f, 0.f, 0.f);
+      *reinterpret_cast<float4*>(&Vs[wv][tok][4 * c4]) = v;
+    }
+    const bool border = wa_regions(p, w, regs[wv], lane);
+    wa_f16x s[2][2];
+    load_bias(s, Bs, lane);
+    {
+      float4 kf[2][4], qf[2][4];
+#pragma unroll
+      for (int t = 0; t < 2; ++t) {
+        const int tok = t * 32 + l31;
+        const bool real = tok < WA_N;
+        const int row = real ? w.row(g, tok) : -1;
+        load_frag(kf[t], p.k, p.qk_ld, row, p.k_pad, real, col0, h, 1.f);
+        load_frag(qf[t], p.q, p.qk_ld, row, p.q_pad, real, col0, h, p.scale);
+      }
+      mma_hd(s, kf, qf);
+    }
+    wave_lds_sync();
+    if (border) {
+#pragma unroll
+      for (int n = 0; n < 2; ++n) {
+        const int rq = regs[wv][n * 32 + l31];
+#pragma unroll
+        for (int t = 0; t < 2; ++t)
+#pragma unroll
+          for (int r = 0; r < 16; ++r)
+            if (regs[wv][t * 32 + acc_row(r, h)] != rq) s[t][n][r] -= 100.f;
+      }
+    }
+    float lse[2];
 #pragma unroll
     for (int n = 0; n < 2; ++n) {
-      const int rq = regs[wv][n * 32 + l31];
+      float m = -INFINITY;
 #pragma unroll
       for (int t = 0; t < 2; ++t)
 #pragma unroll
-        for (int r = 0; r < 16; ++r)
-          if (regs[wv][t * 32 + acc_row(r, h)] != rq) s[t][n][r] -= 100.f;
-    }
-  }
-  float lse[2];
-#pragma unroll
-  for (int n = 0; n < 2; ++n) {
-    float m = -INFINITY;
-#pragma unroll
-    for (int t = 0; t < 2; ++t)
-#pragma unroll
-      for (int r = 0; r < 16; ++r) m = fmaxf(m, s[t][n][r]);
-    m = fmaxf(m, __shfl_xor(m, 32, 64));
-    float l = 0.f;
-#pragma unroll
-    for (int t = 0; t < 2; ++t)
-#pragma unroll
-      for (int r = 0; r < 16; ++r) {
-        const float e = __expf(s[t][n][r] - m);
-        s[t][n][r] = e;
-        l += e;
-      }
-    l += __shfl_xor(l, 32, 64);
-    const float inv = 1.f / l;
-#pragma unroll
-    for (int t = 0; t < 2; ++t)
-#pragma unroll
-      for (int r = 0; r < 16; ++r) s[t][n][r] *= inv;
-    lse[n] = m + __logf(l);
-  }
-  wa_f16x o[2];
-#pragma unroll
-  for (int n = 0; n < 2; ++n)
-#pragma unroll
-    for (int r = 0; r < 16; ++r) o[n][r] = 0.f;
-  mma_tok(o, Vs[wv], s, l31, h);
-#pragma unroll
-  for (int n = 0; n < 2; ++n) {
-    const int q = n * 32 + l31;
-    if (q >= WA_N) continue;
-    const int row = w.row(g, q);
-    if (p.lse && h == 0) p.lse[(int64_t)it.item * WA_N + q] = row >= 0 ? lse[n] : INFINITY;
-    if (row < 0) continue;
-    float* dst = p.out + (int64_t)row * p.out_ld + col0;
-#pragma unroll
-    for (int a = 0; a < 4; ++a)
-      *reinterpret_cast<float4*>(dst + 8 * a + 4 * h) =
-          make_float4(o[n][4 * a], o[n][4 * a + 1], o[n][4 * a + 2], o[n][4 * a + 3]);
-  }
-}
-
-#ifdef WA_OCC3
-constexpr int WA_TR = 56, WA_TP = 57;
-#else
-constexpr int WA_TR = WA_NP, WA_TP = WA_NP + 1;
-#endif
+        for (int r = 0; r < 16; ++r) m = fmaxf(m, s[t][n][r]);
+      m = fmaxf(m, __shfl_xor(m, 32, 64));
+      float l = 0.f;
+#pragma unroll
+      for (int t = 0; t < 2; ++t)
+#pragma unroll
+        for (int r = 0; r < 16; ++r) {
+          const float e = __expf(s[t][n][r] - m);
+          s[t][n][r] = e;
+          l += e;
+        }
+      l += __shfl_xor(l, 32, 64);
+      const float inv = 1.f / l;
+#pragma unroll
+      for (int t = 0; t < 2; ++t)
+#pragma unroll
+        for (int r = 0; r < 16; ++r) s[t][n][r] *= inv;
+      lse[n] = m + __logf(l);
+    }
+    wa_f16x o[2];
+#pragma unroll
+    for (int n = 0; n < 2; ++n)
+#pragma unroll
+      for (int r = 0; r < 16; ++r) o[n][r] = 0.f;
+    mma_tok(o, Vs[wv], s, l31, h);
+#pragma unroll
+    for (int n = 0; n < 2; ++n) {
+      const int q = n * 32 + l31;
+      if (q >= WA_N) continue;
+      const int row = w.row(g, q);
+      if (p.lse && h == 0) p.lse[(int64_t)item * WA_N + q] = row >= 0 ? lse[n] : INFINITY;
+      if (row < 0) continue;
+      float* dst = p.out + (int64_t)row * p.out_ld + col0;
+#pragma unroll
+      for (int a = 0; a < 4; ++a)
+        *reinterpret_cast<float4*>(dst + 8 * a + 4 * h) =
+            make_float4(o[n][4 * a], o[n][4 * a + 1], o[n][4 * a + 2], o[n][4 * a + 3]);
+    }
+  }
+}
+
+constexpr int WA_TR = 56, WA_TP = WA_NP + 1;
+static_assert(WA_TR >= WA_N && WA_TR % 8 == 0, "image rows are dropped by whole accumulator register groups");
 
 __device__ __forceinline__ float col_val(const float* base, int64_t ld, const float* pad, int row, int col) {
-  const float* src = row >= 0 ? base + (int64_t)row * ld + col : ((row == -1 && pad) ? pad + col : g_wa_zero + (col & 31));
+  const float* src =
+      row >= 0 ? base + (int64_t)row * ld + col : ((row == -1 && pad) ? pad + col : g_wa_zero + (col & 31));
   return *src;
 }
 
@@ -315,7 +317,8 @@
           c[t][r] = 0.f;
           continue;
         }
-        const float v = cb[__umul24((unsigned)rt[kind ? t * 32 + acc_row(r, 0) : t * 32 + acc_row(r, h)], (unsigned)ld)];
+        const float v =
+            cb[__umul24((unsigned)rt[kind ? t * 32 + acc_row(r, 0) : t * 32 + acc_row(r, h)], (unsigned)ld)];
         c[t][r] = (kind && h) ? 0.f : v;
       }
   } else {
@@ -327,232 +330,227 @@
 }
 
 template <int WS, int HD>
-#ifdef WA_OCC3
-#define WA_BWD_OCC 3
-#else
-#define WA_BWD_OCC 2
-#endif
-__global__ __launch_bounds__(256) __attribute__((amdgpu_waves_per_eu(WA_BWD_OCC, WA_BWD_OCC))) void winattn_bwd_kernel(
-    WinParams p, const float* __restrict__ biasT, int nitems) {
+__global__ __launch_bounds__(256) __attribute__((amdgpu_waves_per_eu(WA_BWD_WG_PER_CU, WA_BWD_WG_PER_CU))) void
+winattn_bwd_kernel(WinParams p, const float* __restrict__ biasT, int nwin, int slots) {
   __shared__ float tbuf[WA_WAVES][WA_TR][WA_TP];
+  __shared__ float Bs[16][64][4];
   __shared__ float padk[WA_WAVES][WA_HD], padv[WA_WAVES][WA_HD];
   __shared__ int8_t regs[WA_WAVES][WA_NP];
   __shared__ int rowtab[WA_WAVES][WA_NP];
   const WinGeom& g = p.g;
   const int lane = threadIdx.x & 63, wv = threadIdx.x >> 6, l31 = lane & 31, h = lane >> 5;
-  const WaItem it = wa_item(p);
-  if (it.item >= nitems) return;
-  const Win<WS> w(g, it.win);
-  const int col0 = it.hh * HD;
-  if (wa_dead(p, w.b)) {
-    wa_zero_rows(g, w, p.dq, p.dqk_ld, col0, lane);
-    wa_zero_rows(g, w, p.dk, p.dqk_ld, col0, lane);
-    wa_zero_rows(g, w, p.dv, p.dv_ld, col0, lane);
-    float* P = p.partial + (int64_t)it.item * (WA_T + 2 * HD);
-    for (int e = lane; e < WA_T + 2 * HD; e += 64) P[e] = 0.f;
-    return;
-  }
-  float lse[2];
-#pragma unroll
-  for (int n = 0; n < 2; ++n) {
-    const int q = n * 32 + l31;
-    lse[n] = (q < WA_N) ? p.lse[(int64_t)it.item * WA_N + q] : INFINITY;
-  }
-  const int myrow = lane < WA_N ? w.row(g, lane) : -2;
-  rowtab[wv][lane] = myrow;
-  if (lane < HD) { padk[wv][lane] = 0.f; padv[wv][lane] = 0.f; }
-  const bool border = wa_regions(p, w, regs[wv], lane);
-  const bool fast = p.off32 && __ballot(myrow == -1) == 0;
-
-  wa_f16x s[2][2], dp[2][2];
-  load_bias(s, biasT + (size_t)it.hh * 4096, lane);
-  int trow[2];
-  bool treal[2];
-  {
-    float4 kf[2][4], qf[2][4];
-#pragma unroll
-    for (int t = 0; t < 2; ++t) {
-      const int tok = t * 32 + l31;
-      treal[t] = tok < WA_N;
-      trow[t] = treal[t] ? w.row(g, tok) : -1;
-      load_frag(kf[t], p.k, p.qk_ld, trow[t], p.k_pad, treal[t], col0, h, 1.f);
-      load_frag(qf[t], p.q, p.qk_ld, trow[t], p.q_pad, treal[t], col0, h, p.scale);
-    }
-    mma_hd(s, kf, qf);
-  }
-  wave_lds_sync();
-  if (border) {
+  const int hh = wa_head(blockIdx.x, g.heads), slot = wa_slot(blockIdx.x, g.heads);
+  const int col0 = hh * HD;
+  stage_bias(Bs, biasT + (size_t)hh * 4096);
+  __syncthreads();
+  for (int win = wa_first_win(slot, wv); win < nwin; win += wa_win_stride(slots)) {
+    const int item = wa_item_index(win, g.heads, hh);
+    const Win<WS> w(g, win);
+    if (wa_dead(p, w.b)) {
+      wa_zero_rows(g, w, p.dq, p.dqk_ld, col0, lane);
+      wa_zero_rows(g, w, p.dk, p.dqk_ld, col0, lane);
+      wa_zero_rows(g, w, p.dv, p.dv_ld, col0, lane);
+      float* P = p.partial + (int64_t)item * (WA_T + 2 * HD);
+      for (int e = lane; e < WA_T + 2 * HD; e += 64) P[e] = 0.f;
+      continue;
+    }
+    float lse[2];
 #pragma unroll
     for (int n = 0; n < 2; ++n) {
-      const int rq = regs[wv][n * 32 + l31];
+      const int q = n * 32 + l31;
+      lse[n] = (q < WA_N) ? p.lse[(int64_t)item * WA_N + q] : INFINITY;
+    }
+    wave_lds_sync();
+    const int myrow = lane < WA_N ? w.row(g, lane) : -2;
+    rowtab[wv][lane] = myrow;
+    if (lane < HD) { padk[wv][lane] = 0.f; padv[wv][lane] = 0.f; }
+    const bool border = wa_regions(p, w, regs[wv], lane);
+    const bool fast = p.off32 && __ballot(myrow == -1) == 0;
+
+    wa_f16x s[2][2], dp[2][2];
+    load_bias(s, Bs, lane);
+    int trow[2];
+    bool treal[2];
+    {
+      float4 kf[2][4], qf[2][4];
+#pragma unroll
+      for (int t = 0; t < 2; ++t) {
+        const int tok = t * 32 + l31;
+        treal[t] = tok < WA_N;
+        trow[t] = treal[t] ? w.row(g, tok) : -1;
+        load_frag(kf[t], p.k, p.qk_ld, trow[t], p.k_pad, treal[t], col0, h, 1.f);
+        load_frag(qf[t], p.q, p.qk_ld, trow[t], p.q_pad, treal[t], col0, h, p.scale);
+      }
+      mma_hd(s, kf, qf);
+    }
+    wave_lds_sync();
+    if (border) {
+#pragma unroll
+      for (int n = 0; n < 2; ++n) {
+        const int rq = regs[wv][n * 32 + l31];
+#pragma unroll
+        for (int t = 0; t < 2; ++t)
+#pragma unroll
+          for (int r = 0; r < 16; ++r)
+            if (regs[wv][t * 32 + acc_row(r, h)] != rq) s[t][n][r] -= 100.f;
+      }
+    }
+#pragma unroll
+    for (int n = 0; n < 2; ++n)
 #pragma unroll
       for (int t = 0; t < 2; ++t)
 #pragma unroll
-        for (int r = 0; r < 16; ++r)
-          if (regs[wv][t * 32 + acc_row(r, h)] != rq) s[t][n][r] -= 100.f;
-    }
-  }
-#pragma unroll
-  for (int n = 0; n < 2; ++n)
-#pragma unroll
-    for (int t = 0; t < 2; ++t)
-#pragma unroll
-      for (int r = 0; r < 16; ++r) s[t][n][r] = __expf(s[t][n][r] - lse[n]);
-  auto to_lds = [&](const wa_f16x (&x)[2][2]) {
-#pragma unroll
-    for (int t = 0; t < 2; ++t)
+        for (int r = 0; r < 16; ++r) s[t][n][r] = __expf(s[t][n][r] - lse[n]);
+    auto to_lds = [&](const wa_f16x (&x)[2][2]) {
+#pragma unroll
+      for (int t = 0; t < 2; ++t)
+#pragma unroll
+        for (int n = 0; n < 2; ++n)
+#pragma unroll
+          for (int r = 0; r < 16; ++r) {
+            if (t * 32 + acc_row(r, 0) >= WA_TR) continue;
+            tbuf[wv][t * 32 + acc_row(r, h)][n * 32 + l31] = x[t][n][r];
+          }
+    };
+    const int krow[2] = {l31, min(32 + l31, WA_TR - 1)};
+    auto key_side = [&](const float (&colv)[25], float* gbase, int64_t gld, float* padacc) {
+      wa_f16x acc[2];
+#pragma unroll
+      for (int ti = 0; ti < 2; ++ti)
+#pragma unroll
+        for (int r = 0; r < 16; ++r) acc[ti][r] = 0.f;
+#pragma unroll
+      for (int j = 0; j < 25; ++j)
+#pragma unroll
+        for (int ti = 0; ti < 2; ++ti) acc[ti] = mfma32(tbuf[wv][krow[ti]][2 * j + h], colv[j], acc[ti]);
+      if (fast) {
+        float* gb = gbase + col0 + l31;
+        const int* rt = rowtab[wv];
+#pragma unroll
+        for (int ti = 0; ti < 2; ++ti)
+#pragma unroll
+          for (int r = 0; r < 16; ++r) {
+            const int kind = acc_tok_kind(ti, r);
+            if (kind == 2 || (kind == 1 && h)) continue;
+            gb[__umul24((unsigned)rt[ti * 32 + acc_row(r, h)], (unsigned)gld)] = acc[ti][r];
+          }
+        return;
+      }
+#pragma unroll
+      for (int ti = 0; ti < 2; ++ti)
+#pragma unroll
+        for (int r = 0; r < 16; ++r) {
+          const int row = rowtab[wv][ti * 32 + acc_row(r, h)];
+          if (row >= 0) gbase[(int64_t)row * gld + col0 + l31] = acc[ti][r];
+          else if (row == -1) atomicAdd(&padacc[l31], acc[ti][r]);
+        }
+    };
+    {
+      to_lds(s);
+      wave_lds_sync();
+      float dc[25];
+      if (fast) fetch_pairs<true>(dc, p.dout, p.out_ld, nullptr, rowtab[wv], col0, l31, h, 1.f);
+      else fetch_pairs<false>(dc, p.dout, p.out_ld, nullptr, rowtab[wv], col0, l31, h, 1.f);
+      key_side(dc, p.dv, p.dv_ld, padv[wv]);
+    }
+    float D[2];
+    {
+      float4 vf[2][4], df[2][4];
+#pragma unroll
+      for (int t = 0; t < 2; ++t) {
+        const bool qo = treal[t] && trow[t] >= 0;
+        load_frag(vf[t], p.v, p.v_ld, trow[t], p.v_pad, treal[t], col0, h, 1.f);
+        load_frag(df[t], p.dout, p.out_ld, trow[t], nullptr, qo, col0, h, 1.f);
+        float4 of[4];
+        load_frag(of, p.out, p.out_ld, trow[t], nullptr, qo, col0, h, 1.f);
+        float part = 0.f;
+#pragma unroll
+        for (int g4 = 0; g4 < 4; ++g4) part += dot4(df[t][g4], of[g4]);
+        D[t] = part + __shfl_xor(part, 32, 64);
+      }
+#pragma unroll
+      for (int a = 0; a < 2; ++a)
+#pragma unroll
+        for (int b = 0; b < 2; ++b)
+#pragma unroll
+          for (int r = 0; r < 16; ++r) dp[a][b][r] = 0.f;
+      mma_hd(dp, vf, df);
+    }
+#pragma unroll
+    for (int n = 0; n < 2; ++n)
+#pragma unroll
+      for (int t = 0; t < 2; ++t)
+#pragma unroll
+        for (int r = 0; r < 16; ++r) {
+          float pr = 0.f;
+          if (t * 32 + acc_row(r, 0) < WA_TR) pr = tbuf[wv][t * 32 + acc_row(r, h)][n * 32 + l31];
+          dp[t][n][r] = pr * (dp[t][n][r] - D[n]);
+        }
+    float kc[2][16];
+    if (fast) fetch_keys<true>(kc, p.k, p.qk_ld, p.k_pad, rowtab[wv], col0, l31, h);
+    else fetch_keys<false>(kc, p.k, p.qk_ld, p.k_pad, rowtab[wv], col0, l31, h);
+    wave_lds_sync();
+    to_lds(dp);
+    wave_lds_sync();
+    float qc[25];
+    if (fast) fetch_pairs<true>(qc, p.q, p.qk_ld, p.q_pad, rowtab[wv], col0, l31, h, p.scale);
+    else fetch_pairs<false>(qc, p.q, p.qk_ld, p.q_pad, rowtab[wv], col0, l31, h, p.scale);
+    {
+      wa_f16x dq[2];
 #pragma unroll
       for (int n = 0; n < 2; ++n)
 #pragma unroll
-        for (int r = 0; r < 16; ++r) {
-#ifdef WA_OCC3
-          if (t * 32 + acc_row(r, 0) >= WA_TR || (n == 1 && l31 >= WA_TP - 32)) continue;
-#endif
-          tbuf[wv][t * 32 + acc_row(r, h)][n * 32 + l31] = x[t][n][r];
-        }
-  };
-  auto key_side = [&](const float (&colv)[25], float* gbase, int64_t gld, float* padacc) {
-    wa_f16x acc[2];
-#pragma unroll
-    for (int ti = 0; ti < 2; ++ti)
-#pragma unroll
-      for (int r = 0; r < 16; ++r) acc[ti][r] = 0.f;
-#pragma unroll
-    for (int j = 0; j < 25; ++j)
-#pragma unroll
-      for (int ti = 0; ti < 2; ++ti) acc[ti] = mfma32(tbuf[wv][ti * 32 + l31][2 * j + h], colv[j], acc[ti]);
-    if (fast) {
-      float* gb = gbase + col0 + l31;
-      const int* rt = rowtab[wv];
-#pragma unroll
-      for (int ti = 0; ti < 2; ++ti)
-#pragma unroll
-        for (int r = 0; r < 16; ++r) {
-          const int kind = acc_tok_kind(ti, r);
-          if (kind == 2 || (kind == 1 && h)) continue;
-          gb[__umul24((unsigned)rt[ti * 32 + acc_row(r, h)], (unsigned)gld)] = acc[ti][r];
-        }
-      return;
-    }
-#pragma unroll
-    for (int ti = 0; ti < 2; ++ti)
-#pragma unroll
-      for (int r = 0; r < 16; ++r) {
-        const int row = rowtab[wv][ti * 32 + acc_row(r, h)];
-        if (row >= 0) gbase[(int64_t)row * gld + col0 + l31] = acc[ti][r];
-        else if (row == -1) atomicAdd(&padacc[l31], acc[ti][r]);
-      }
-  };
-  {
-    to_lds(s);
+        for (int r = 0; r < 16; ++r) dq[n][r] = 0.f;
+#pragma unroll
+      for (int t = 0; t < 2; ++t)
+#pragma unroll
+        for (int r = 0; r < (t == 0 ? 16 : 12); ++r)
+#pragma unroll
+          for (int n = 0; n < 2; ++n)
+            dq[n] = mfma32(kc[t][r], tbuf[wv][t * 32 + acc_row(r, h)][n * 32 + l31], dq[n]);
+#pragma unroll
+      for (int n = 0; n < 2; ++n) {
+        if (!treal[n] || trow[n] < 0) continue;
+        float* dst = p.dq + (int64_t)trow[n] * p.dqk_ld + col0;
+#pragma unroll
+        for (int a = 0; a < 4; ++a)
+          *reinterpret_cast<float4*>(dst + 8 * a + 4 * h) =
+              make_float4(dq[n][4 * a] * p.scale, dq[n][4 * a + 1] * p.scale, dq[n][4 * a + 2] * p.scale,
+                          dq[n][4 * a + 3] * p.scale);
+      }
+    }
+    key_side(qc, p.dk, p.dqk_ld, padk[wv]);
+    float E[13];
+#pragma unroll
+    for (int e = 0; e < 13; ++e) E[e] = 0.f;
+    const int sky = lane / WS, sqy = lane - sky * WS;
+    if (lane < WA_N) {
+      const float* blk = &tbuf[wv][sky * WS][sqy * WS];
+#pragma unroll
+      for (int kx = 0; kx < WS; ++kx)
+#pragma unroll
+        for (int qx = 0; qx < WS; ++qx) E[qx - kx + WS - 1] += blk[kx * WA_TP + qx];
+    }
     wave_lds_sync();
-    float dc[25];
-    if (fast) fetch_pairs<true>(dc, p.dout, p.out_ld, nullptr, rowtab[wv], col0, l31, h, 1.f);
-    else fetch_pairs<false>(dc, p.dout, p.out_ld, nullptr, rowtab[wv], col0, l31, h, 1.f);
-    key_side(dc, p.dv, p.dv_ld, padv[wv]);
-  }
-  float D[2];
-  {
-    float4 vf[2][4], df[2][4];
-#pragma unroll
-    for (int t = 0; t < 2; ++t) {
-      const bool qo = treal[t] && trow[t] >= 0;
-      load_frag(vf[t], p.v, p.v_ld, trow[t], p.v_pad, treal[t], col0, h, 1.f);
-      load_frag(df[t], p.dout, p.out_ld, trow[t], nullptr, qo, col0, h, 1.f);
-      float4 of[4];
-      load_frag(of, p.out, p.out_ld, trow[t], nullptr, qo, col0, h, 1.f);
-      float part = 0.f;
-#pragma unroll
-      for (int g4 = 0; g4 < 4; ++g4) part += dot4(df[t][g4], of[g4]);
-      D[t] = part + __shfl_xor(part, 32, 64);
-    }
-#pragma unroll
-    for (int a = 0; a < 2; ++a)
-#pragma unroll
-      for (int b = 0; b < 2; ++b)
-#pragma unroll
-        for (int r = 0; r < 16; ++r) dp[a][b][r] = 0.f;
-    mma_hd(dp, vf, df);
-  }
-#pragma unroll
-  for (int n = 0; n < 2; ++n)
-#pragma unroll
-    for (int t = 0; t < 2; ++t)
-#pragma unroll
-      for (int r = 0; r < 16; ++r) {
-        float pr;
-#ifdef WA_OCC3
-        if (t * 32 + acc_row(r, 0) >= WA_TR) pr = 0.f;
-        else if (n == 1) pr = l31 < WA_TP - 32 ? tbuf[wv][t * 32 + acc_row(r, h)][32 + min(l31, WA_TP - 33)] : 0.f;
-        else
-#endif
-        pr = tbuf[wv][t * 32 + acc_row(r, h)][n * 32 + l31];
-        dp[t][n][r] = pr * (dp[t][n][r] - D[n]);
-      }
-  float kc[2][16];
-  if (fast) fetch_keys<true>(kc, p.k, p.qk_ld, p.k_pad, rowtab[wv], col0, l31, h);
-  else fetch_keys<false>(kc, p.k, p.qk_ld, p.k_pad, rowtab[wv], col0, l31, h);
-  wave_lds_sync();
-  to_lds(dp);
-  wave_lds_sync();
-  float qc[25];
-  if (fast) fetch_pairs<true>(qc, p.q, p.qk_ld, p.q_pad, rowtab[wv], col0, l31, h, p.scale);
-  else fetch_pairs<false>(qc, p.q, p.qk_ld, p.q_pad, rowtab[wv], col0, l31, h, p.scale);
-  {
-    wa_f16x dq[2];
-#pragma unroll
-    for (int n = 0; n < 2; ++n)
-#pragma unroll
-      for (int r = 0; r < 16; ++r) dq[n][r] = 0.f;
-#pragma unroll
-    for (int t = 0; t < 2; ++t)
-#pragma unroll
-      for (int r = 0; r < (t == 0 ? 16 : 12); ++r)
-#pragma unroll
-        for (int n = 0; n < 2; ++n)
-          dq[n] = mfma32(kc[t][r], tbuf[wv][t * 32 + acc_row(r, h)][n * 32 + l31], dq[n]);
-#pragma unroll
-    for (int n = 0; n < 2; ++n) {
-      if (!treal[n] || trow[n] < 0) continue;
-      float* dst = p.dq + (int64_t)trow[n] * p.dqk_ld + col0;
-#pragma unroll
-      for (int a = 0; a < 4; ++a)
-        *reinterpret_cast<float4*>(dst + 8 * a + 4 * h) =
-            make_float4(dq[n][4 * a] * p.scale, dq[n][4 * a + 1] * p.scale, dq[n][4 * a + 2] * p.scale,
-                        dq[n][4 * a + 3] * p.scale);
-    }
-  }
-  key_side(qc, p.dk, p.dqk_ld, padk[wv]);
-  float E[13];
-#pragma unroll
-  for (int e = 0; e < 13; ++e) E[e] = 0.f;
-  const int sky = lane / WS, sqy = lane - sky * WS;
-  if (lane < WA_N) {
-    const float* blk = &tbuf[wv][sky * WS][sqy * WS];
-#pragma unroll
-    for (int kx = 0; kx < WS; ++kx)
-#pragma unroll
-      for (int qx = 0; qx < WS; ++qx) E[qx - kx + WS - 1] += blk[kx * WA_TP + qx];
-  }
-  wave_lds_sync();
-  constexpr int ND = 2 * WS - 1;
-  float* Eb = &tbuf[wv][0][0];
-  if (lane < WA_N) {
-#pragma unroll
-    for (int e = 0; e < ND; ++e) Eb[lane * ND + e] = E[e];
-  }
-  wave_lds_sync();
-  float* P = p.partial + (int64_t)it.item * (WA_T + 2 * HD);
-  for (int e = lane; e < WA_T; e += 64) {
-    const int dy = e / ND - (WS - 1), dxi = e % ND;
-    const int ky0 = max(0, -dy), ky1 = min(WS - 1, WS - 1 - dy);
-    float acc = 0.f;
-    for (int ky = ky0; ky <= ky1; ++ky) acc += Eb[(ky * WS + ky + dy) * ND + dxi];
-    P[e] = acc;
-  }
-  if (lane < HD) {
-    P[WA_T + lane] = padk[wv][lane];
-    P[WA_T + HD + lane] = padv[wv][lane];
+    constexpr int ND = 2 * WS - 1;
+    float* Eb = &tbuf[wv][0][0];
+    if (lane < WA_N) {
+#pragma unroll
+      for (int e = 0; e < ND; ++e) Eb[lane * ND + e] = E[e];
+    }
+    wave_lds_sync();
+    float* P = p.partial + (int64_t)item * (WA_T + 2 * HD);
+    for (int e = lane; e < WA_T; e += 64) {
+      const int dy = e / ND - (WS - 1), dxi = e % ND;
+      const int ky0 = max(0, -dy), ky1 = min(WS - 1, WS - 1 - dy);
+      float acc = 0.f;
+      for (int ky = ky0; ky <= ky1; ++ky) acc += Eb[(ky * WS + ky + dy) * ND + dxi];
+      P[e] = acc;
+    }
+    if (lane < HD) {
+      P[WA_T + lane] = padk[wv][lane];
+      P[WA_T + HD + lane] = padv[wv][lane];
+    }
   }
 }
 
@@ -615,6 +613,7 @@
     for (int64_t ld : lds) ok = ok && ld >= 0 && ld < (1 << 24) && rows * ld < (int64_t(1) << 32);
     p.off32 = ok;
   }
+  MDEMI_REQUIRE((int64_t)d->B * p.g.nWh * p.g.nWw < (int64_t(1) << 30), "winattn: too many windows");
   nwin = d->B * p.g.nWh * p.g.nWw;
   return MDEMI_OK;
 }
@@ -624,6 +623,25 @@
 using namespace mdemi;
 
 static int wa_items(const mdemi_winattn_desc* d, int nwin) { return nwin * d->heads; }
+
+static int wa_device_cus() {
+  static int cus[64] = {0};
+  int dev = 0;
+  if (hipGetDevice(&dev) != hipSuccess || dev < 0 || dev >= 64) return 256;
+  if (!cus[dev]) {
+    hipDeviceProp_t pr;
+    cus[dev] = hipGetDeviceProperties(&pr, dev) == hipSuccess && pr.multiProcessorCount > 0 ? pr.multiProcessorCount
+                                                                                           : 256;
+  }
+  return cus[dev];
+}
+
+static int g_wa_max_wg = 0;
+extern "C" void mdemi_winattn_set_max_workgroups(int n) { g_wa_max_wg = n > 0 ? n : 0; }
+
+static WaPlan wa_launch_plan(const mdemi_winattn_desc* d, int nwin, int wg_per_cu) {
+  return wa_plan(nwin, d->heads, wa_default_max_wg(wa_device_cus(), wg_per_cu, g_wa_max_wg));
+}
 static size_t wa_bias_bytes(const mdemi_winattn_desc* d) { return (size_t)d->heads * 4096 * sizeof(float); }
 
 extern "C" size_t mdemi_winattn_fwd_workspace_size(const mdemi_winattn_desc* d) {
@@ -647,9 +665,9 @@
   float* biasT = (float*)d->workspace;
   hipLaunchKernelGGL(wa_bias_kernel, dim3(d->heads * 16), dim3(256), 0, st, d->rpb_table, d->heads, biasT,
                      (float*)nullptr);
-  const int nitems = wa_items(d, nwin);
-  hipLaunchKernelGGL((winattn_fwd_kernel<7, 32>), dim3(cdiv(nitems, WA_WAVES)), dim3(64 * WA_WAVES), 0, st, p,
-                     (const float*)biasT, nitems);
+  const WaPlan pl = wa_launch_plan(d, nwin, WA_FWD_WG_PER_CU);
+  hipLaunchKernelGGL((winattn_fwd_kernel<7, 32>), dim3((unsigned)pl.grid), dim3(64 * WA_WAVES), 0, st, p,
+                     (const float*)biasT, pl.nwin, pl.slots);
   return check_launch("winattn_fwd");
 }
 
@@ -694,8 +712,9 @@
   else
     hipLaunchKernelGGL(wa_bias_kernel, dim3(d->heads * 16), dim3(256), 0, st, d->rpb_table, d->heads, biasT,
                        (float*)nullptr);
-  hipLaunchKernelGGL((winattn_bwd_kernel<7, 32>), dim3((unsigned)cdiv(items, WA_WAVES)), dim3(64 * WA_WAVES), 0, st,
-                     p, (const float*)biasT, items);
+  const WaPlan pl = wa_launch_plan(d, nwin, WA_BWD_WG_PER_CU);
+  hipLaunchKernelGGL((winattn_bwd_kernel<7, 32>), dim3((unsigned)pl.grid), dim3(64 * WA_WAVES), 0, st, p,
+                     (const float*)biasT, pl.nwin, pl.slots);
   int rc2 = colsum_launch(p.partial, nwin, (int64_t)d->heads * R, (int64_t)d->heads * R, sums, 0, cws, st);
   if (rc2) return rc2;
   hipLaunchKernelGGL((winattn_bwd_scatter<7, 32>), dim3((d->heads * R + 255) / 256), dim3(256), 0, st, sums, d->heads,
diff --git a/monocular-depth-estimation_amd/mdemi/_lib.py b/monocular-depth-estimation_amd/mdemi/_lib.py
--- a/monocular-depth-estimation_amd/mdemi/_lib.py
+++ b/monocular-depth-estimation_amd/mdemi/_lib.py
@@ -166,6 +166,7 @@
     "mdemi_winattn_bwd_workspace_size": (sz, [ctypes.POINTER(WinAttnDesc)]),
     "mdemi_winattn_bwd": (ctypes.c_int, [ctypes.POINTER(WinAttnDesc), vp]),
     "mdemi_winattn_bwd_bias": (ctypes.c_int, [ctypes.POINTER(WinAttnDesc), vp, vp]),
+    "mdemi_winattn_set_max_workgroups": (None, [ctypes.c_int]),
     "mdemi_silog_workspace_size": (sz, [i32, i64]),
     "mdemi_silog_fwd": (ctypes.c_int, [vp, vp, vp, vp, i32, i64, f32, f32, f32, i32, i32, vp, vp]),
     "mdemi_silog_bwd": (ctypes.c_int, [vp, vp, vp, vp, vp, i32, i64, f32, f32, f32, i32, i32, vp]),
```

New measurement: 63.19 images/sec, median of 6. No clear change (+0.1%).
